# wustl-cig/FLAIR

Hardware: AMD Instinct MI355X
Metric: restored frames/sec at 256x256, 16-frame clip, 250-step DDIM (higher is better)
Workload: dtype bf16

## Files before the change

flair_amd/csrc/api.hip:

```cpp
#include <stdarg.h>
#include <stdio.h>

#include "common.h"

static thread_local char g_err[512] = "";

void flair_set_error(const char* fmt, ...) {
    va_list ap;
    va_start(ap, fmt);
    vsnprintf(g_err, sizeof(g_err), fmt, ap);
    va_end(ap);
}

extern "C" const char* flair_last_error(void) { return g_err; }
extern "C" int flair_abi_version(void) { return 11; }

#include <dlfcn.h>

typedef int (*flair_nccl_bcast_fn)(const void*, void*, size_t, int, int, void*, hipStream_t);

extern "C" int flair_bcast_weights(void* blob, size_t bytes, int root, void* rccl_comm, hipStream_t stream) {
    FLAIR_CHECK(blob && bytes > 0 && rccl_comm && root >= 0, "flair_bcast_weights: bad argument (blob, bytes, root, communicator)");
    static flair_nccl_bcast_fn fn = nullptr;
    if (!fn) {
        void* h = nullptr;
        for (const char* name : {"librccl.so", "librccl.so.1"}) {
            h = dlopen(name, RTLD_NOW | RTLD_NOLOAD);
            if (!h) h = dlopen(name, RTLD_NOW | RTLD_GLOBAL);
            if (h) break;
        }
        FLAIR_CHECK(h, "flair_bcast_weights: librccl.so not found (%s)", dlerror());
        fn = reinterpret_cast<flair_nccl_bcast_fn>(dlsym(h, "ncclBroadcast"));
        FLAIR_CHECK(fn, "flair_bcast_weights: ncclBroadcast not found in librccl");
    }
    const size_t chunk = (size_t)512 << 20;
    for (size_t off = 0; off < bytes; off += chunk) {
        const size_t n = bytes - off < chunk ? bytes - off : chunk;
        char* p = reinterpret_cast<char*>(blob) + off;
        const int rc = fn(p, p, n,  1, root, rccl_comm, stream);
        if (rc != 0) {
            flair_set_error("flair_bcast_weights: ncclBroadcast returned %d", rc);
            return FLAIR_ERR_HIP;
        }
    }
    return FLAIR_OK;
}

namespace {
typedef __attribute__((ext_vector_type(8))) __bf16 probe_bf16x8;
typedef __attribute__((ext_vector_type(16))) float probe_f32x16;

__global__ __launch_bounds__(256) void probe_matrix_kernel(float* sink, int iters) {
    probe_f32x16 acc[4];
    for (int i = 0; i < 4; ++i)
        for (int r = 0; r < 16; ++r) acc[i][r] = 0.f;
    probe_bf16x8 a, b;
    for (int e = 0; e < 8; ++e) {
        a[e] = (__bf16)(0.001f * (float)((threadIdx.x + e) & 255));
        b[e] = (__bf16)(0.002f * (float)((threadIdx.x + 2 * e) & 255));
    }
    for (int it = 0; it < iters; ++it) {
#pragma unroll
        for (int u = 0; u < 4; ++u)
#pragma unroll
            for (int i = 0; i < 4; ++i) acc[i] = __builtin_amdgcn_mfma_f32_32x32x16_bf16(a, b, acc[i], 0, 0, 0);
    }
    float s = 0.f;
    for (int i = 0; i < 4; ++i)
        for (int r = 0; r < 16; ++r) s += acc[i][r];
    if (s == 12345.678f) sink[0] = s;
}

__global__ __launch_bounds__(256) void probe_stream_kernel(const uint4* __restrict__ src, uint4* __restrict__ dst, size_t n, int mode) {
    unsigned sum = 0;
    for (size_t i = blockIdx.x * (size_t)blockDim.x + threadIdx.x; i < n; i += (size_t)gridDim.x * blockDim.x) {
        if (mode == 1) {
            dst[i] = make_uint4((unsigned)i, 1u, 2u, 3u);
        } else {
            const uint4 v = src[i];
            if (mode == 2) dst[i] = v;
            else sum ^= v.x ^ v.y ^ v.z ^ v.w;
        }
    }
    if (mode == 0 && sum == 0x12345679u) dst[0] = make_uint4(sum, 0u, 0u, 0u);
}
}

extern "C" int flair_probe_matrix_rate(int iters, int workgroups_per_cu, float* sink, double* flop_out, hipStream_t stream) {
    FLAIR_CHECK(iters > 0 && workgroups_per_cu >= 1 && workgroups_per_cu <= 8 && sink, "flair_probe_matrix_rate: bad argument");
    const int grid = flair_cu_count() * workgroups_per_cu;
    hipLaunchKernelGGL(probe_matrix_kernel, dim3(grid), dim3(256), 0, stream, sink, iters);
    FLAIR_LAUNCH_CHECK();
    if (flop_out) *flop_out = (double)grid * 4  * iters * 16  * (2.0 * 32 * 32 * 16);
    return FLAIR_OK;
}

extern "C" int flair_probe_stream_rate(const void* src, void* dst, size_t bytes, int mode, hipStream_t stream) {
    FLAIR_CHECK(dst && (mode == 1 || src) && bytes >= 16 && mode >= 0 && mode <= 2, "flair_probe_stream_rate: bad argument (mode 0 read, 1 write, 2 copy)");
    FLAIR_CHECK((reinterpret_cast<uintptr_t>(dst) & 15) == 0 && (reinterpret_cast<uintptr_t>(src) & 15) == 0, "flair_probe_stream_rate: 16-byte aligned buffers");
    hipLaunchKernelGGL(probe_stream_kernel, dim3(flair_cu_count() * 8), dim3(256), 0, stream, reinterpret_cast<const uint4*>(src),
                       reinterpret_cast<uint4*>(dst), bytes / 16, mode);
    FLAIR_LAUNCH_CHECK();
    return FLAIR_OK;
}
```

flair_amd/csrc/common.h:

```cpp
#pragma once
#include <hip/hip_runtime.h>
#include <stdint.h>

#include "../../include/flair_hip.h"

typedef __attribute__((ext_vector_type(8))) __bf16 bf16x8;
typedef __attribute__((ext_vector_type(16))) float f32x16;
typedef __attribute__((ext_vector_type(4))) float f32x4;

typedef uint16_t bf16_t;

#define FLAIR_WAVE 64

void flair_set_error(const char* fmt, ...);
#define FLAIR_CHECK(cond, ...)            \
    do {                                  \
        if (!(cond)) {                    \
            flair_set_error(__VA_ARGS__); \
            return FLAIR_ERR_ARG;         \
        }                                 \
    } while (0)
#define FLAIR_CHECK_VIEW(fn, name, ptr, ld, C, vec)                                                                   \
    FLAIR_CHECK((ld) >= (C) && (ld) % (vec) == 0 && reinterpret_cast<uintptr_t>(ptr) % 16 == 0,                        \
                fn ": " name " stride/alignment: " name "_ld = %d must be >= C = %d and a multiple of %d elements, " \
                name " = %p 16-byte aligned", (int)(ld), (int)(C), (int)(vec), (const void*)(ptr))
#define FLAIR_LAUNCH_CHECK()                                                  \
    do {                                                                      \
        hipError_t e_ = hipGetLastError();                                    \
        if (e_ != hipSuccess) {                                               \
            flair_set_error("HIP launch failed: %s", hipGetErrorString(e_));  \
            return FLAIR_ERR_HIP;                                             \
        }                                                                     \
    } while (0)

__device__ __forceinline__ float bf2f(bf16_t v) {
    return __uint_as_float(((uint32_t)v) << 16);
}
__device__ __forceinline__ bf16_t f2bf(float f) {
    __bf16 b = (__bf16)f;
    return __builtin_bit_cast(bf16_t, b);
}
__device__ __forceinline__ uint32_t pack2bf(float lo, float hi) {
    return (uint32_t)f2bf(lo) | ((uint32_t)f2bf(hi) << 16);
}

template <typename E> struct ET;
template <> struct ET<float> {
    static constexpr int VEC = 4;
    static constexpr int DT = FLAIR_F32;
    static __device__ __forceinline__ float ld(const float* p) { return *p; }
    static __device__ __forceinline__ void st(float* p, float v) { *p = v; }
};
template <> struct ET<bf16_t> {
    static constexpr int VEC = 8;
    static constexpr int DT = FLAIR_BF16;
    static __device__ __forceinline__ float ld(const bf16_t* p) { return bf2f(*p); }
    static __device__ __forceinline__ void st(bf16_t* p, float v) { *p = f2bf(v); }
};

template <typename E> struct Vec16;
template <> struct Vec16<float> {
    static __device__ __forceinline__ void load(const float* p, float* o) {
        float4 v = *reinterpret_cast<const float4*>(p);
        o[0] = v.x; o[1] = v.y; o[2] = v.z; o[3] = v.w;
    }
    static __device__ __forceinline__ void store(float* p, const float* o) {
        *reinterpret_cast<float4*>(p) = make_float4(o[0], o[1], o[2], o[3]);
    }
};
template <> struct Vec16<bf16_t> {
    static __device__ __forceinline__ void load(const bf16_t* p, float* o) {
        uint4 v = *reinterpret_cast<const uint4*>(p);
        o[0] = __uint_as_float(v.x << 16); o[1] = __uint_as_float(v.x & 0xffff0000u);
        o[2] = __uint_as_float(v.y << 16); o[3] = __uint_as_float(v.y & 0xffff0000u);
        o[4] = __uint_as_float(v.z << 16); o[5] = __uint_as_float(v.z & 0xffff0000u);
        o[6] = __uint_as_float(v.w << 16); o[7] = __uint_as_float(v.w & 0xffff0000u);
    }
    static __device__ __forceinline__ void store(bf16_t* p, const float* o) {
        uint4 v;
        v.x = pack2bf(o[0], o[1]); v.y = pack2bf(o[2], o[3]);
        v.z = pack2bf(o[4], o[5]); v.w = pack2bf(o[6], o[7]);
        *reinterpret_cast<uint4*>(p) = v;
    }
};

__device__ __forceinline__ float silu_f(float v) { return v / (1.0f + __expf(-v)); }

__device__ __forceinline__ float apply_act(float v, int act) {
    switch (act) {
        case FLAIR_ACT_RELU: return v > 0.f ? v : 0.f;
        case FLAIR_ACT_LRELU01: return v > 0.f ? v : 0.1f * v;
        case FLAIR_ACT_SILU: return silu_f(v);
        case FLAIR_ACT_LRELU02: return v > 0.f ? v : 0.2f * v;
        case FLAIR_ACT_GELU: return 0.5f * v * (1.f + erff(v * 0.70710678118654752f));
        default: return v;
    }
}

template <int N>
__device__ __forceinline__ void dcn_offset_act(float (&v)[N], int co, float mag, int period) {
    const bool residue = 3 * (co % period) < 2 * period;
#pragma unroll
    for (int e = 0; e < N; ++e) {
        const float r = __builtin_amdgcn_rcpf(1.f + __expf(residue ? 2.f * v[e] : -v[e]));
        v[e] = residue ? mag * (1.f - 2.f * r) : r;
    }
}

template <int N>
__device__ __forceinline__ void dcn_offset_act_fast(float (&v)[N], int co, float mag, int period, float scale) {
    const bool residue = 3 * (co % period) < 2 * period;
    const float kk = residue ? 2.885390081777927f : -1.4426950408889634f;
    const float A = residue ? -2.f * mag * scale : scale, B = residue ? mag * scale : 0.f;
#pragma unroll
    for (int e = 0; e < N; ++e) v[e] = fmaf(__builtin_amdgcn_rcpf(1.f + __builtin_amdgcn_exp2f(kk * v[e])), A, B);
}

typedef __attribute__((ext_vector_type(4))) unsigned int u32x4_t;
#define FLAIR_OOB 0x80000000u
__device__ __forceinline__ __amdgpu_buffer_rsrc_t make_rsrc(const void* p, unsigned bytes) {
    return __builtin_amdgcn_make_buffer_rsrc(const_cast<void*>(p), 0, (int)bytes, 0x00020000);
}
__device__ __forceinline__ uint4 buf_load16(__amdgpu_buffer_rsrc_t r, unsigned byteOff) {
    const u32x4_t v = __builtin_amdgcn_raw_buffer_load_b128(r, (int)byteOff, 0, 0);
    return make_uint4(v.x, v.y, v.z, v.w);
}

__device__ __forceinline__ int xcd_remap(int bid, int nwg) {
    const int q = nwg >> 3, r = nwg & 7, xcd = bid & 7;
    const int base = xcd < r ? xcd * (q + 1) : r * (q + 1) + (xcd - r) * q;
    return base + (bid >> 3);
}

template <int NBYTES>
__device__ __forceinline__ void prefetch_kernargs() {
#ifdef FLAIR_NO_KARG_PREFETCH
    return;
#endif
    const auto ka = __builtin_amdgcn_kernarg_segment_ptr();
    constexpr int LINES = (NBYTES + 63) / 64 + 1;
    unsigned t0, t1, t2, t3, t4, t5, t6, t7;
    if constexpr (LINES <= 2)
        asm volatile("s_load_dword %0, %2, 0x0\n\ts_load_dword %1, %2, 0x40\n\ts_waitcnt lgkmcnt(0)" : "=&s"(t0), "=&s"(t1) : "s"(ka) : "memory");
    else if constexpr (LINES <= 4)
        asm volatile("s_load_dword %0, %4, 0x0\n\ts_load_dword %1, %4, 0x40\n\ts_load_dword %2, %4, 0x80\n\ts_load_dword %3, %4, 0xc0\n\t"
                     "s_waitcnt lgkmcnt(0)" : "=&s"(t0), "=&s"(t1), "=&s"(t2), "=&s"(t3) : "s"(ka) : "memory");
    else if constexpr (LINES <= 6)
        asm volatile("s_load_dword %0, %6, 0x0\n\ts_load_dword %1, %6, 0x40\n\ts_load_dword %2, %6, 0x80\n\ts_load_dword %3, %6, 0xc0\n\t"
                     "s_load_dword %4, %6, 0x100\n\ts_load_dword %5, %6, 0x140\n\ts_waitcnt lgkmcnt(0)"
                     : "=&s"(t0), "=&s"(t1), "=&s"(t2), "=&s"(t3), "=&s"(t4), "=&s"(t5) : "s"(ka) : "memory");
    else
        asm volatile("s_load_dword %0, %8, 0x0\n\ts_load_dword %1, %8, 0x40\n\ts_load_dword %2, %8, 0x80\n\ts_load_dword %3, %8, 0xc0\n\t"
                     "s_load_dword %4, %8, 0x100\n\ts_load_dword %5, %8, 0x140\n\ts_load_dword %6, %8, 0x180\n\ts_load_dword %7, %8, 0x1c0\n\t"
                     "s_waitcnt lgkmcnt(0)"
                     : "=&s"(t0), "=&s"(t1), "=&s"(t2), "=&s"(t3), "=&s"(t4), "=&s"(t5), "=&s"(t6), "=&s"(t7) : "s"(ka) : "memory");
}

__device__ __forceinline__ void dma16(u32x4_t desc, unsigned voff, unsigned ldsAddr) {
    unsigned keep;
    asm volatile("s_mov_b32 %0, m0\n\ts_mov_b32 m0, %2\n\ts_nop 0\n\tbuffer_load_dwordx4 %1, %3, 0 offen lds\n\ts_mov_b32 m0, %0"
                 : "=&s"(keep)
                 : "v"(voff), "s"(ldsAddr), "s"(desc)
                 : "memory");
}

__device__ __forceinline__ u32x4_t make_desc(const void* base, unsigned bytes) {
    const unsigned long long b = reinterpret_cast<unsigned long long>(base);
    u32x4_t d;
    d.x = __builtin_amdgcn_readfirstlane((unsigned)b);
    d.y = __builtin_amdgcn_readfirstlane((unsigned)(b >> 32) & 0xffffu);
    d.z = __builtin_amdgcn_readfirstlane(bytes);
    d.w = 0x00020000u;
    return d;
}

struct LdsAttrOnce {
    unsigned long long done = 0;
};
static inline hipError_t flair_max_lds_once(LdsAttrOnce& st, const void* fn, int bytes = 160 * 1024) {
    int dev = 0;
    if (hipGetDevice(&dev) != hipSuccess) dev = -1;
    if (dev >= 0 && dev < 64 && ((st.done >> dev) & 1ull)) return hipSuccess;
    const hipError_t e = hipFuncSetAttribute(fn, hipFuncAttributeMaxDynamicSharedMemorySize, bytes);
    if (e == hipSuccess && dev >= 0 && dev < 64) st.done |= 1ull << dev;
    return e;
}
static inline int flair_cu_count() {
    static int cus[64] = {};
    int dev = 0;
    if (hipGetDevice(&dev) != hipSuccess || dev < 0 || dev >= 64) return 256;
    if (!cus[dev]) {
        hipDeviceProp_t prop;
        cus[dev] = hipGetDeviceProperties(&prop, dev) == hipSuccess && prop.multiProcessorCount > 0 ? prop.multiProcessorCount : 256;
    }
    return cus[dev];
}

static inline int cdiv(long a, long b) { return (int)((a + b - 1) / b); }
```

flair_amd/csrc/conv.hip:

```cpp
#include <type_traits>

#include "common.h"

namespace {

struct ConvArgs {
    const void* x[4];
    int segC[4];
    int segLd[4];
    int nseg;
    const void* w;
    const float* bias;
    const void* res0;
    const void* res1;
    int res0Ld, res1Ld;
    void* y;
    int yLd;
    int T, H, W;
    int KT, KH, KW;
    int Cout, CinTot;
    int act;
    float outScale;
    long P;
    int nPixTiles, nCoTiles;
    int tFast;
    unsigned segBytes[4];
    unsigned wBytes;
    float* part;
    int splitK;
    const float* fbias;
    int fbiasLd;
    int stride;
    int tapShift;
    int reflect;
    float actParam;
    int actPeriod;
    int Hin, Win;
    int esz;
};

template <typename E> struct Mma;

template <> struct Mma<bf16_t> {
    static constexpr int BKE = 32;
    static __device__ __forceinline__ int chunk(int i, int half) { return 2 * i + half; }
    static __device__ __forceinline__ void run(const uint4 (&a)[2], const uint4 (&b)[2], f32x16& acc) {
        acc = __builtin_amdgcn_mfma_f32_32x32x16_bf16(__builtin_bit_cast(bf16x8, a[0]),
                                                      __builtin_bit_cast(bf16x8, b[0]), acc, 0, 0, 0);
        acc = __builtin_amdgcn_mfma_f32_32x32x16_bf16(__builtin_bit_cast(bf16x8, a[1]),
                                                      __builtin_bit_cast(bf16x8, b[1]), acc, 0, 0, 0);
    }
    static __device__ __forceinline__ void run1(const uint4& a, const uint4& b, f32x16& acc) {
        acc = __builtin_amdgcn_mfma_f32_32x32x16_bf16(__builtin_bit_cast(bf16x8, a), __builtin_bit_cast(bf16x8, b),
                                                      acc, 0, 0, 0);
    }
    static constexpr int MFMA_PER_HALF = 1;
};

template <> struct Mma<float> {
    static constexpr int BKE = 16;
    static __device__ __forceinline__ int chunk(int i, int half) { return 2 * half + i; }
    static __device__ __forceinline__ void run(const uint4 (&a)[2], const uint4 (&b)[2], f32x16& acc) {
        const float* af = reinterpret_cast<const float*>(a);
        const float* bf = reinterpret_cast<const float*>(b);
#pragma unroll
        for (int s = 0; s < 8; ++s)
            acc = __builtin_amdgcn_mfma_f32_32x32x2f32(af[s], bf[s], acc, 0, 0, 0);
    }
    static __device__ __forceinline__ void run1(const uint4& a, const uint4& b, f32x16& acc) {
        const float* af = reinterpret_cast<const float*>(&a);
        const float* bf = reinterpret_cast<const float*>(&b);
#pragma unroll
        for (int s = 0; s < 4; ++s)
            acc = __builtin_amdgcn_mfma_f32_32x32x2f32(af[s], bf[s], acc, 0, 0, 0);
    }
    static constexpr int MFMA_PER_HALF = 4;
};

__device__ __forceinline__ int lds_off(int row, int chunk) {
    return row * 64 + ((chunk ^ ((row >> 2) & 3)) << 4);
}

__device__ __forceinline__ int staged_row(int id) {
    const int g = id >> 3;
    return (g >> 2) * 8 + (g & 3) + 4 * ((id >> 2) & 1);
}

template <typename E>
__device__ __forceinline__ void store_quad(const ConvArgs& a, long p, int co, float v0, float v1, float v2, float v3) {
    if (co >= a.Cout) return;
    float v[4] = {v0, v1, v2, v3};
    if (a.bias) {
        const float4 b = *reinterpret_cast<const float4*>(a.bias + co);
        v[0] += b.x; v[1] += b.y; v[2] += b.z; v[3] += b.w;
    }
    if (a.fbias) {
        const float* fb = a.fbias + (p / ((long)a.H * a.W)) * a.fbiasLd + co;
        v[0] += fb[0]; v[1] += fb[1]; v[2] += fb[2]; v[3] += fb[3];
    }
    if (a.act == FLAIR_ACT_DCN_OFFSETS) {
        dcn_offset_act<4>(v, co, a.actParam, a.actPeriod);
    } else {
#pragma unroll
        for (int e = 0; e < 4; ++e) v[e] = apply_act(v[e], a.act);
    }
    const E* r0 = reinterpret_cast<const E*>(a.res0);
    const E* r1 = reinterpret_cast<const E*>(a.res1);
    if (r0) {
#pragma unroll
        for (int e = 0; e < 4; ++e) v[e] += ET<E>::ld(r0 + p * a.res0Ld + co + e);
    }
    if (r1) {
#pragma unroll
        for (int e = 0; e < 4; ++e) v[e] += ET<E>::ld(r1 + p * a.res1Ld + co + e);
    }
#pragma unroll
    for (int e = 0; e < 4; ++e) v[e] *= a.outScale;
    E* dst = reinterpret_cast<E*>(a.y) + p * a.yLd + co;
    if constexpr (sizeof(E) == 4) {
        *reinterpret_cast<float4*>(dst) = make_float4(v[0], v[1], v[2], v[3]);
    } else {
        uint2 pk;
        pk.x = pack2bf(v[0], v[1]);
        pk.y = pack2bf(v[2], v[3]);
        *reinterpret_cast<uint2*>(dst) = pk;
    }
}

template <typename E, int ACT, int FC, int FP>
__device__ __forceinline__ void igemm_epilogue(const ConvArgs& a, const f32x16 (&acc)[FC][FP], long pbase, int cobase, int lr, int lh) {
    constexpr unsigned ESZ = sizeof(E);
    constexpr int VEC = ET<E>::VEC, NV = 8 / VEC;
    const float slope = a.act == FLAIR_ACT_NONE ? 1.f : a.act == FLAIR_ACT_RELU ? 0.f : a.act == FLAIR_ACT_LRELU01 ? 0.1f : 0.2f;
    const unsigned yLdB = (unsigned)a.yLd * ESZ, r0LdB = (unsigned)a.res0Ld * ESZ, r1LdB = (unsigned)a.res1Ld * ESZ;
    constexpr unsigned SPAN = FP * 32;
    const __amdgpu_buffer_rsrc_t yd = make_rsrc(reinterpret_cast<char*>(a.y) + ((size_t)pbase * a.yLd + cobase) * ESZ, SPAN * yLdB);
    const __amdgpu_buffer_rsrc_t r0d = make_rsrc(reinterpret_cast<const char*>(a.res0) + (a.res0 ? ((size_t)pbase * a.res0Ld + cobase) * ESZ : 0),
                                                 a.res0 ? SPAN * r0LdB : 0u);
    const __amdgpu_buffer_rsrc_t r1d = make_rsrc(reinterpret_cast<const char*>(a.res1) + (a.res1 ? ((size_t)pbase * a.res1Ld + cobase) * ESZ : 0),
                                                 a.res1 ? SPAN * r1LdB : 0u);
    const int coLeft = a.Cout - cobase;
    const __amdgpu_buffer_rsrc_t bd = make_rsrc(a.bias ? a.bias + cobase : nullptr, a.bias && coLeft > 0 ? (unsigned)coLeft * 4u : 0u);
    const long hw = (long)a.H * a.W;
#pragma unroll
    for (int j = 0; j < FP; ++j) {
        const long p = pbase + j * 32 + lr;
        const bool pvalid = p < a.P;
        const unsigned pl = (unsigned)(j * 32 + lr);
        const float* fbrow = a.fbias ? a.fbias + (pvalid ? p / hw : 0) * a.fbiasLd + cobase : nullptr;
#pragma unroll
        for (int i = 0; i < FC; ++i) {
            uint4 bq[2][2], r0v[2][NV], r1v[2][NV], fq[2][2];
#pragma unroll
            for (int jj = 0; jj < 2; ++jj) {
                const int cw = i * 32 + 16 * jj + 8 * lh;
                const bool ok = pvalid && cw < coLeft;
                bq[jj][0] = buf_load16(bd, 4u * (unsigned)cw);
                bq[jj][1] = buf_load16(bd, 4u * (unsigned)cw + 16u);
#pragma unroll
                for (int q = 0; q < NV; ++q) {
                    r0v[jj][q] = buf_load16(r0d, ok ? pl * r0LdB + (unsigned)(cw + q * VEC) * ESZ : FLAIR_OOB);
                    r1v[jj][q] = buf_load16(r1d, ok ? pl * r1LdB + (unsigned)(cw + q * VEC) * ESZ : FLAIR_OOB);
                }
                fq[jj][0] = fq[jj][1] = make_uint4(0u, 0u, 0u, 0u);
            }
            if (a.fbias) {
#pragma unroll
                for (int jj = 0; jj < 2; ++jj) {
                    const int cw = i * 32 + 16 * jj + 8 * lh;
                    const float* fp = fbrow + (cw < coLeft ? cw : 0);
                    fq[jj][0] = *reinterpret_cast<const uint4*>(fp);
                    fq[jj][1] = *reinterpret_cast<const uint4*>(fp + 4);
                }
            }
#pragma unroll
            for (int jj = 0; jj < 2; ++jj) {
                const f32x16& c = acc[i][j];
                float v[8];
#pragma unroll
                for (int e = 0; e < 4; ++e) {
                    const auto sw2 = __builtin_amdgcn_permlane32_swap(__float_as_uint(c[8 * jj + e]), __float_as_uint(c[8 * jj + 4 + e]), false, false);
                    v[e] = __uint_as_float(sw2[0]);
                    v[4 + e] = __uint_as_float(sw2[1]);
                }
                const int cw = i * 32 + 16 * jj + 8 * lh;
                const bool ok = pvalid && cw < coLeft;
                {
                    const uint4 b0 = bq[jj][0], b1 = bq[jj][1], f0 = fq[jj][0], f1 = fq[jj][1];
                    v[0] += __uint_as_float(b0.x) + __uint_as_float(f0.x); v[1] += __uint_as_float(b0.y) + __uint_as_float(f0.y);
                    v[2] += __uint_as_float(b0.z) + __uint_as_float(f0.z); v[3] += __uint_as_float(b0.w) + __uint_as_float(f0.w);
                    v[4] += __uint_as_float(b1.x) + __uint_as_float(f1.x); v[5] += __uint_as_float(b1.y) + __uint_as_float(f1.y);
                    v[6] += __uint_as_float(b1.z) + __uint_as_float(f1.z); v[7] += __uint_as_float(b1.w) + __uint_as_float(f1.w);
                }
// ... 157 lines not shown
            fa0[set][0] = *reinterpret_cast<const uint4*>(wb0 + tap9 * PITCH + 16 * Mma<E>::chunk(0, lh));
            fa0[set][1] = *reinterpret_cast<const uint4*>(wb0 + tap9 * PITCH + 16 * Mma<E>::chunk(1, lh));
            fa1[set][0] = *reinterpret_cast<const uint4*>(wb1 + tap9 * PITCH + 16 * Mma<E>::chunk(0, lh));
            fa1[set][1] = *reinterpret_cast<const uint4*>(wb1 + tap9 * PITCH + 16 * Mma<E>::chunk(1, lh));
#pragma unroll
            for (int j = 0; j < RPW; ++j) {
                const char* hp = hb + ((j + kh) * HW_ + kw) * PITCH;
                fb[set][j][0] = *reinterpret_cast<const uint4*>(hp + 16 * Mma<E>::chunk(0, lh));
                fb[set][j][1] = *reinterpret_cast<const uint4*>(hp + 16 * Mma<E>::chunk(1, lh));
            }
        };
        load_tap(0, 0);
        __builtin_amdgcn_sched_group_barrier(0x100, 4 + 2 * RPW, 0);
#pragma unroll
        for (int tap9 = 0; tap9 < 9; ++tap9) {
            const int set = tap9 & 1;
            if (tap9 < 8) load_tap(set ^ 1, tap9 + 1);
#pragma unroll
            for (int j = 0; j < RPW; ++j) {
                Mma<E>::run(fa0[set], fb[set][j], acc[j][0]);
                Mma<E>::run(fa1[set], fb[set][j], acc[j][1]);
            }
            if (tap9 < 8) __builtin_amdgcn_sched_group_barrier(0x100, 4 + 2 * RPW, 0);
            __builtin_amdgcn_sched_group_barrier(0x8, (sizeof(E) == 2 ? 4 : 16) * RPW, 0);
        }
    };

    int issued = 0;
#pragma unroll
    for (int s_ = 0; s_ < PF; ++s_)
        if (issued < nch) {
            issue(hreg[s_], wreg[s_]);
            advance();
            ++issued;
        }
    write_lds(hreg[0], wreg[0]);
    __syncthreads();
    for (int k = 0; k < nch; k += PF) {
#pragma unroll
        for (int par = 0; par < PF; ++par) {
            const int kk = k + par;
            if (kk < nch) {
                if (issued < nch) {
                    issue(hreg[par], wreg[par]);
                    advance();
                    ++issued;
                }
                compute();
                if (kk + 1 < nch) {
                    __syncthreads();
                    write_lds(hreg[(par + 1) % PF], wreg[(par + 1) % PF]);
                    __syncthreads();
                }
            }
        }
    }

    if ((a.Cout & 7) == 0) {
        constexpr int VEC = ET<E>::VEC;
        constexpr int CHUNKS = 64 / VEC;
        __syncthreads();
#pragma unroll
        for (int j = 0; j < RPW; ++j) {
            char* tile = smem + (wave * RPW + j) * 32 * (64 * 4 + 16);
#pragma unroll
            for (int i = 0; i < 2; ++i)
#pragma unroll
                for (int g = 0; g < 4; ++g)
                    *reinterpret_cast<float4*>(tile + lr * (64 * 4 + 16) + (i * 32 + 8 * g + 4 * lh) * 4) =
                        make_float4(acc[j][i][4 * g], acc[j][i][4 * g + 1], acc[j][i][4 * g + 2],
                                    acc[j][i][4 * g + 3]);
        }
        __syncthreads();
        constexpr int FPITCH = 64 * 4 + 16;
#pragma unroll
        for (int j = 0; j < RPW; ++j) {
            const int h = h0 + wave * RPW + j;
            if (h >= a.H) continue;
            const char* tile = smem + (wave * RPW + j) * 32 * FPITCH;
            const long prow = ((long)t * a.H + h) * a.W + w0;
#pragma unroll
            for (int it = 0; it < 32 * CHUNKS / 64; ++it) {
                const int id = it * 64 + lane;
                const int px = id / CHUNKS, ch = id % CHUNKS;
                const int co = co0 + ch * VEC;
                if (co >= a.Cout) continue;
                const long p = prow + px;
                float v[VEC];
                const float* src = reinterpret_cast<const float*>(tile + px * FPITCH) + ch * VEC;
#pragma unroll
                for (int e = 0; e < VEC; e += 4) {
                    const float4 q = *reinterpret_cast<const float4*>(src + e);
                    v[e] = q.x; v[e + 1] = q.y; v[e + 2] = q.z; v[e + 3] = q.w;
                }
                if (a.bias) {
#pragma unroll
                    for (int e = 0; e < VEC; ++e) v[e] += a.bias[co + e];
                }
                if (a.fbias) {
                    const float* fb = a.fbias + (long)t * a.fbiasLd + co;
#pragma unroll
                    for (int e = 0; e < VEC; ++e) v[e] += fb[e];
                }
                if (a.act == FLAIR_ACT_DCN_OFFSETS) {
                    dcn_offset_act<VEC>(v, co, a.actParam, a.actPeriod);
                } else {
#pragma unroll
                    for (int e = 0; e < VEC; ++e) v[e] = apply_act(v[e], a.act);
                }
                if (a.res0) {
                    float r[VEC];
                    Vec16<E>::load(reinterpret_cast<const E*>(a.res0) + p * a.res0Ld + co, r);
#pragma unroll
                    for (int e = 0; e < VEC; ++e) v[e] += r[e];
                }
                if (a.res1) {
                    float r[VEC];
                    Vec16<E>::load(reinterpret_cast<const E*>(a.res1) + p * a.res1Ld + co, r);
#pragma unroll
                    for (int e = 0; e < VEC; ++e) v[e] += r[e];
                }
#pragma unroll
                for (int e = 0; e < VEC; ++e) v[e] *= a.outScale;
                Vec16<E>::store(reinterpret_cast<E*>(a.y) + p * a.yLd + co, v);
            }
        }
        return;
    }
#pragma unroll
    for (int j = 0; j < RPW; ++j) {
        const int h = h0 + wave * RPW + j, w = w0 + lr;
        if (h >= a.H) continue;
        const long p = ((long)t * a.H + h) * a.W + w;
#pragma unroll
        for (int i = 0; i < 2; ++i)
#pragma unroll
            for (int g = 0; g < 4; ++g)
                store_quad<E>(a, p, co0 + i * 32 + 8 * g + 4 * lh, acc[j][i][4 * g], acc[j][i][4 * g + 1],
                              acc[j][i][4 * g + 2], acc[j][i][4 * g + 3]);
    }
}

template <typename E, int TH, int RPW, int PF>
int launch_halo(const ConvArgs& a0, hipStream_t s) {
    ConvArgs a = a0;
    a.nCoTiles = cdiv(a.Cout, 64);
    const int grid = a.T * cdiv(a.H, TH) * (a.W / 32) * a.nCoTiles;
    const size_t lds = (size_t)(TH + 2) * 34 * 80 + 64 * 9 * 80;
    hipLaunchKernelGGL((conv3x3_halo_kernel<E, TH, RPW, PF>), dim3(grid), dim3(64 * TH / RPW), lds, s, a);
    FLAIR_LAUNCH_CHECK();
    return FLAIR_OK;
}

template <typename E, int TH, int RPW, int CF>
__global__ __launch_bounds__(256 * TH / RPW / CF, (256 * TH / RPW / CF) / 256) void conv3x3_halo_ks_kernel(ConvArgs a) {
    static_assert(RPW == 1 && CF == 2, "one image row and both 32-cout fragments per wave");
    prefetch_kernargs<sizeof(ConvArgs)>();
    constexpr int NRG = TH / RPW;
    constexpr int NCG = 2 / CF;
    constexpr int NW = 2 * NRG * NCG, NT = 64 * NW;
    constexpr int BKE = Mma<E>::BKE;
    constexpr int VEC = ET<E>::VEC;
    constexpr unsigned ESZ = sizeof(E);
    constexpr int HW_ = 34, PITCH = 80;
    constexpr int HALO_ROWS = (TH + 2) * HW_;
    constexpr int HALO_PIECES = (HALO_ROWS + 7) / 8 * 8 * 4;
    constexpr int W_PIECES = 64 * 9 * 4;
    constexpr int HI = (HALO_PIECES + NT - 1) / NT;
    constexpr int WI = (W_PIECES + NT - 1) / NT;
    constexpr int HALO_BYTES = (TH + 2) * HW_ * PITCH;
    constexpr int STAGE_BYTES = HALO_BYTES + 64 * 9 * PITCH;
    extern __shared__ __attribute__((aligned(16))) char smem[];

    const int tid = threadIdx.x, lane = tid & 63, wave = tid >> 6;
    const int lr = lane & 31, lh = lane >> 5;
    const int rp = wave % NRG, kh2 = (wave / NRG) & 1, cg = wave / (2 * NRG);
    const int bid = xcd_remap(blockIdx.x, gridDim.x);
    const int coTile = bid % a.nCoTiles;
    int rest = bid / a.nCoTiles;
    const int tilesW = a.W / 32, tilesH = (a.H + TH - 1) / TH;
    const int tw = rest % tilesW;
    rest /= tilesW;
    const int th = rest % tilesH;
    const int t = rest / tilesH;
    const int h0 = th * TH, w0 = tw * 32, co0 = coTile * 64;
    const int taps = a.KT * 9;
    const int pt = a.KT / 2;

    float biasv[VEC];
    {
        const int bco = co0 + (lane % (64 / VEC)) * VEC;
#pragma unroll
        for (int e = 0; e < VEC; ++e) biasv[e] = (a.bias && bco < a.Cout) ? a.bias[bco + e] : 0.f;
    }
    uint4 hreg[HI], wreg[WI];
    int dt = -pt, seg = 0, cb = 0, segOff = 0;
    auto dt_valid = [&](int d) { return (unsigned)(t + d) < (unsigned)a.T; };
    while (dt <= pt && !dt_valid(dt)) ++dt;

    int hpix[HI];
    unsigned hq[HI], woff[WI];
#pragma unroll
    for (int i = 0; i < HI; ++i) {
        const int id = i * NT + tid;
        const int pix = staged_row(id);
        const int r = pix / HW_, c = pix % HW_;
        const int hh = h0 + r - 1, ww = w0 + c - 1;
        const bool ok = pix < HALO_ROWS && (unsigned)hh < (unsigned)a.H && (unsigned)ww < (unsigned)a.W;
        hpix[i] = ok ? hh * a.W + ww : -1;
        hq[i] = (id & 3) * VEC * ESZ;
    }
    const __amdgpu_buffer_rsrc_t wrs = make_rsrc(a.w, a.wBytes);
#pragma unroll
    for (int i = 0; i < WI; ++i) {
        const int id = i * NT + tid;
        const int row = staged_row(id);
        const int co = row / 9, tap9 = row % 9;
        const bool ok = id < W_PIECES && co0 + co < a.Cout;
        woff[i] = ok ? (unsigned)(((co0 + co) * taps + tap9) * a.CinTot + (id & 3) * VEC) * ESZ : FLAIR_OOB;
    }
    auto issue = [&]() {
        const unsigned ld = (unsigned)a.segLd[seg] * ESZ;
        const char* frame = reinterpret_cast<const char*>(a.x[seg]) + (size_t)(t + dt) * a.H * a.W * ld;
        const __amdgpu_buffer_rsrc_t xr = make_rsrc(frame, a.segBytes[seg]);
        const unsigned cofs = (unsigned)(cb * BKE) * ESZ;
#pragma unroll
        for (int i = 0; i < HI; ++i)
            hreg[i] = buf_load16(xr, hpix[i] >= 0 ? (unsigned)hpix[i] * ld + cofs + hq[i] : FLAIR_OOB);
        const unsigned kofs = (unsigned)((dt + pt) * 9 * a.CinTot + segOff + cb * BKE) * ESZ;
#pragma unroll
        for (int i = 0; i < WI; ++i) wreg[i] = buf_load16(wrs, woff[i] == FLAIR_OOB ? FLAIR_OOB : woff[i] + kofs);
        ++cb;
        if (cb * BKE >= a.segC[seg]) {
            cb = 0;
            segOff += a.segC[seg];
            if (++seg >= a.nseg) {
                seg = 0;
                segOff = 0;
                ++dt;
                while (dt <= pt && !dt_valid(dt)) ++dt;
            }
        }
    };
    auto write_lds = [&](int stage) {
        char* sh = smem + stage * STAGE_BYTES;
        char* sw = sh + HALO_BYTES;
#pragma unroll
        for (int i = 0; i < HI; ++i) {
            const int id = i * NT + tid;
            const int row = staged_row(id);
            if (row < HALO_ROWS) *reinterpret_cast<uint4*>(sh + row * PITCH + (id & 3) * 16) = hreg[i];
        }
#pragma unroll
        for (int i = 0; i < WI; ++i) {
            const int id = i * NT + tid;
            if (id < W_PIECES) *reinterpret_cast<uint4*>(sw + staged_row(id) * PITCH + (id & 3) * 16) = wreg[i];
        }
    };
    int nValidDt = 0;
    for (int d = -pt; d <= pt; ++d) nValidDt += dt_valid(d) ? 1 : 0;
    const int nch = nValidDt * (a.CinTot / BKE);

    f32x16 acc[RPW][CF];
#pragma unroll
    for (int j = 0; j < RPW; ++j)
#pragma unroll
        for (int i = 0; i < CF; ++i)
#pragma unroll
            for (int r = 0; r < 16; ++r) acc[j][i][r] = 0.f;

    const int ck = 16 * Mma<E>::chunk(kh2, lh);
    auto compute = [&](int stage) {
        const char* sh = smem + stage * STAGE_BYTES;
        const char* hb = sh + ((RPW * rp * HW_) + lr) * PITCH + ck;
        const char* wb0 = sh + HALO_BYTES + ((cg * CF * 32 + lr) * 9) * PITCH + ck;
        uint4 fa[2][CF], fb[2][RPW];
        auto load_tap = [&](int set, int tap9) {
            const int kh = tap9 / 3, kw = tap9 % 3;
#pragma unroll
            for (int i = 0; i < CF; ++i)
                fa[set][i] = *reinterpret_cast<const uint4*>(wb0 + (i * 32 * 9 + tap9) * PITCH);
#pragma unroll
            for (int j = 0; j < RPW; ++j)
                fb[set][j] = *reinterpret_cast<const uint4*>(hb + ((kh + j) * HW_ + kw) * PITCH);
        };
        load_tap(0, 0);
        __builtin_amdgcn_sched_group_barrier(0x100, CF + RPW, 0);
#pragma unroll
        for (int tap9 = 0; tap9 < 9; ++tap9) {
            const int set = tap9 & 1;
            if (tap9 < 8) load_tap(set ^ 1, tap9 + 1);
#pragma unroll
            for (int j = 0; j < RPW; ++j)
#pragma unroll
                for (int i = 0; i < CF; ++i) Mma<E>::run1(fa[set][i], fb[set][j], acc[j][i]);
            if (tap9 < 8) __builtin_amdgcn_sched_group_barrier(0x100, CF + RPW, 0);
            __builtin_amdgcn_sched_group_barrier(0x8, CF * RPW * Mma<E>::MFMA_PER_HALF, 0);
        }
    };

    issue();
    write_lds(0);
    if (nch > 1) issue();
    __syncthreads();
    for (int k = 0; k < nch; ++k) {
        compute(k & 1);
        if (k + 1 < nch) {
            write_lds((k + 1) & 1);
            if (k + 2 < nch) issue();
            __syncthreads();
        }
    }

    constexpr int FPITCH = 64 * 4 + 16;
    constexpr int CHUNKS = 64 / VEC;
    constexpr int PARTS = NW / TH;
    constexpr int NIT = 32 * CHUNKS / 64 / PARTS;
    const int orow = wave % TH, part = wave / TH;
    const int h = h0 + orow;
    const long prow = ((long)t * a.H + h) * a.W + w0;
    const int ech = lane % CHUNKS;
    const int eco = co0 + ech * VEC;
    const bool eok = h < a.H && eco < a.Cout;
    uint4 r0v[NIT], r1v[NIT];
#pragma unroll
    for (int k = 0; k < NIT; ++k) {
        const int px = ((k * PARTS + part) * 64 + lane) / CHUNKS;
        const long p = prow + px;
        r0v[k] = r1v[k] = make_uint4(0u, 0u, 0u, 0u);
        if (eok && a.res0) r0v[k] = *reinterpret_cast<const uint4*>(reinterpret_cast<const E*>(a.res0) + p * a.res0Ld + eco);
        if (eok && a.res1) r1v[k] = *reinterpret_cast<const uint4*>(reinterpret_cast<const E*>(a.res1) + p * a.res1Ld + eco);
    }
    __syncthreads();
#pragma unroll
    for (int pass = 0; pass < 2; ++pass) {
        if (kh2 == pass) {
#pragma unroll
            for (int j = 0; j < RPW; ++j) {
                char* tile = smem + (RPW * rp + j) * 32 * FPITCH + lr * FPITCH;
#pragma unroll
                for (int i = 0; i < CF; ++i)
#pragma unroll
                    for (int g = 0; g < 4; ++g) {
                        float4* dst = reinterpret_cast<float4*>(tile + ((cg * CF + i) * 32 + 8 * g + 4 * lh) * 4);
                        float4 v = make_float4(acc[j][i][4 * g], acc[j][i][4 * g + 1], acc[j][i][4 * g + 2],
                                               acc[j][i][4 * g + 3]);
                        if (pass == 1) {
                            const float4 o = *dst;
                            v.x += o.x; v.y += o.y; v.z += o.z; v.w += o.w;
                        }
                        *dst = v;
                    }
            }
        }
        __syncthreads();
    }
    if (!eok) return;
    const float slope = a.act == FLAIR_ACT_NONE ? 1.f : a.act == FLAIR_ACT_RELU ? 0.f : a.act == FLAIR_ACT_LRELU01 ? 0.1f : 0.2f;
    const bool leaky = a.act == FLAIR_ACT_NONE || a.act == FLAIR_ACT_RELU || a.act == FLAIR_ACT_LRELU01 || a.act == FLAIR_ACT_LRELU02;
    const char* tile = smem + orow * 32 * FPITCH;
#pragma unroll
    for (int k = 0; k < NIT; ++k) {
        const int px = ((k * PARTS + part) * 64 + lane) / CHUNKS;
        const long p = prow + px;
        float v[VEC];
        const float* src = reinterpret_cast<const float*>(tile + px * FPITCH) + ech * VEC;
#pragma unroll
        for (int e = 0; e < VEC; e += 4) {
            const float4 q = *reinterpret_cast<const float4*>(src + e);
            v[e] = q.x; v[e + 1] = q.y; v[e + 2] = q.z; v[e + 3] = q.w;
        }
#pragma unroll
        for (int e = 0; e < VEC; ++e) v[e] += biasv[e];
        if (a.fbias) {
            const float* fb = a.fbias + (long)t * a.fbiasLd + eco;
#pragma unroll
            for (int e = 0; e < VEC; ++e) v[e] += fb[e];
        }
        if (leaky) {
#pragma unroll
            for (int e = 0; e < VEC; ++e) v[e] = fmaxf(v[e], v[e] * slope);
        } else if (a.act == FLAIR_ACT_DCN_OFFSETS) {
            dcn_offset_act<VEC>(v, eco, a.actParam, a.actPeriod);
        } else if (a.act == FLAIR_ACT_SILU) {
#pragma unroll
            for (int e = 0; e < VEC; ++e) v[e] = silu_f(v[e]);
        } else {
#pragma unroll
            for (int e = 0; e < VEC; ++e) v[e] = apply_act(v[e], a.act);
        }
        if (a.res0) {
            float r[VEC];
            Vec16<E>::load(reinterpret_cast<const E*>(&r0v[k]), r);
#pragma unroll
            for (int e = 0; e < VEC; ++e) v[e] += r[e];
        }
        if (a.res1) {
            float r[VEC];
            Vec16<E>::load(reinterpret_cast<const E*>(&r1v[k]), r);
#pragma unroll
            for (int e = 0; e < VEC; ++e) v[e] += r[e];
        }
#pragma unroll
        for (int e = 0; e < VEC; ++e) v[e] *= a.outScale;
        Vec16<E>::store(reinterpret_cast<E*>(a.y) + p * a.yLd + eco, v);
    }
}

template <typename E, int TH, int RPW, int CF>
int launch_halo_ks(const ConvArgs& a0, hipStream_t s) {
    ConvArgs a = a0;
    a.nCoTiles = cdiv(a.Cout, 64);
    const int grid = a.T * cdiv(a.H, TH) * (a.W / 32) * a.nCoTiles;
    const size_t lds = 2 * ((size_t)(TH + 2) * 34 * 80 + 64 * 9 * 80);
    static LdsAttrOnce attr;
    {
        const hipError_t e = flair_max_lds_once(attr, reinterpret_cast<const void*>(&conv3x3_halo_ks_kernel<E, TH, RPW, CF>));
        FLAIR_CHECK(e == hipSuccess, "flair_conv_nhwc: hipFuncSetAttribute: %s", hipGetErrorString(e));
    }
    hipLaunchKernelGGL((conv3x3_halo_ks_kernel<E, TH, RPW, CF>), dim3(grid), dim3(256 * TH / RPW / CF), lds, s, a);
    FLAIR_LAUNCH_CHECK();
    return FLAIR_OK;
}

struct DmaTile {
    int t, h0, w0, co0;
};

template <int NW, int RPW, int NSTAGE>
__device__ __forceinline__ void conv3x3_dma_body(const ConvArgs& a, int nTiles, int tilesPerXcd) {
    using E = bf16_t;
    static_assert((RPW == 1 || RPW == 2) && NSTAGE == 2, "the clip-level and one-tile forms (two stages)");
    constexpr int KSTEPS = 2;
    constexpr int TH = NW * RPW, HWP = 34;
    constexpr int HALO_ROWS = (TH + 2) * HWP;
    constexpr int HALO_INSTR = (HALO_ROWS + 15) / 16;
    constexpr int W_INSTR = 64 * 9 / 16;
    constexpr int HALO_BYTES = HALO_INSTR * 1024;
    constexpr int STAGE_BYTES = HALO_BYTES + W_INSTR * 1024;
    constexpr int NSLOT = (HALO_INSTR + W_INSTR + NW - 1) / NW;
    constexpr int BIAS_OFF = NSTAGE * STAGE_BYTES + NW * 1024;
    extern __shared__ __attribute__((aligned(16))) char smem[];

    const int tid = threadIdx.x, lane = tid & 63;
    const int wave = __builtin_amdgcn_readfirstlane(tid >> 6);
    const int lr = lane & 31, lh = lane >> 5;
    const int taps = a.KT * 9, pt = a.KT / 2;
    const int chunksPerTap = a.CinTot / 32;
    const int H = a.H, W = a.W, T = a.T;

    const int xcd = blockIdx.x & 7, slot = blockIdx.x >> 3, slotsPerXcd = gridDim.x >> 3;
    const int tilesW = W / 32, tilesH = H / TH, nCoTiles = a.nCoTiles;
    auto tile_at = [&](int i, DmaTile& tl) -> bool {
        const int inXcd = slot + i * slotsPerXcd;
        const int id = xcd * tilesPerXcd + inXcd;
        if (inXcd >= tilesPerXcd || id >= nTiles) return false;
        int rest = id;
        tl.co0 = (rest % nCoTiles) * 64;
        rest /= nCoTiles;
        if (a.tFast) {
            tl.t = rest % T;
            rest /= T;
            tl.w0 = (rest % tilesW) * 32;
            tl.h0 = (rest / tilesW) * TH;
            return true;
        }
        tl.w0 = (rest % tilesW) * 32;
        rest /= tilesW;
        tl.h0 = (rest % tilesH) * TH;
        tl.t = rest / tilesH;
        return true;
    };

    const int lrow = lane >> 2, lchunk = lane & 3;
    unsigned slotv[NSLOT], hchunk[NSLOT];
#pragma unroll
    for (int i = 0; i < NSLOT; ++i) {
        const int id = wave * NSLOT + i;
        const int c = (id * 16 + lrow) % HWP;
        hchunk[i] = (unsigned)((lchunk ^ ((c >> 2) & 3)) << 4);
    }
    auto setup_tile = [&](const DmaTile& tl) {
#pragma unroll
        for (int i = 0; i < NSLOT; ++i) {
            const int id = wave * NSLOT + i;
            const int R = id * 16 + lrow;
            const int hr = R / HWP, c = R - hr * HWP;
            const int hh = tl.h0 - 1 + hr, ww = tl.w0 - 1 + c;
            const bool okh = R < HALO_ROWS && (unsigned)hh < (unsigned)H && (unsigned)ww < (unsigned)W;
            const unsigned hv = okh ? (unsigned)(hh * W + ww) : 0xffffffffu;
            const int row = R - HALO_INSTR * 16;
            const int tap9 = row >> 6, co = row & 63;
            const bool okw = row >= 0 && row < 576 && tl.co0 + co < a.Cout;
            const unsigned wv = okw ? (unsigned)(((tl.co0 + co) * taps + tap9) * a.CinTot) * 2u + ((lchunk ^ ((co >> 2) & 3)) << 4) : FLAIR_OOB;
            slotv[i] = id >= HALO_INSTR ? wv : hv;
        }
    };

    const u32x4_t wdesc = make_desc(a.w, a.wBytes);
    struct Walk {
        int dt, seg, cb, segOff, j;
    };
    auto dt_at = [&](int t, int j) { return a.tFast ? (j + a.KT * T - t) % a.KT - pt : j - pt; };
    auto walk_first = [&](int t, Walk& wk) {
        wk.j = 0; wk.seg = 0; wk.cb = 0; wk.segOff = 0;
        while (wk.j < a.KT && (unsigned)(t + dt_at(t, wk.j)) >= (unsigned)T) ++wk.j;
        wk.dt = dt_at(t, wk.j);
    };
    auto walk_next = [&](int t, Walk& wk) {
        ++wk.cb;
        if (wk.cb * 32 >= a.segC[wk.seg]) {
            wk.cb = 0;
            wk.segOff += a.segC[wk.seg];
            if (++wk.seg >= a.nseg) {
                wk.seg = 0;
                wk.segOff = 0;
                ++wk.j;
                while (wk.j < a.KT && (unsigned)(t + dt_at(t, wk.j)) >= (unsigned)T) ++wk.j;
                wk.dt = dt_at(t, wk.j);
            }
        }
    };
    auto chunks_of = [&](int t) {
        int n = 0;
        for (int d = -pt; d <= pt; ++d) n += (unsigned)(t + d) < (unsigned)T ? 1 : 0;
        return n * chunksPerTap;
    };
    auto issue = [&](const DmaTile& tl, const Walk& wk, int stage) {
        const unsigned ld = (unsigned)a.segLd[wk.seg] * 2u;
        const char* frame = reinterpret_cast<const char*>(a.x[wk.seg]) + (size_t)(tl.t + wk.dt) * H * W * ld;
        const u32x4_t xdesc = make_desc(frame, a.segBytes[wk.seg]);
        const unsigned cofs = (unsigned)(wk.cb * 64);
        const unsigned kofs = (unsigned)((wk.dt + pt) * 9 * a.CinTot + wk.segOff + wk.cb * 32) * 2u;
        const unsigned sbase = (unsigned)(stage * STAGE_BYTES + wave * NSLOT * 1024);
#pragma unroll
        for (int i = 0; i < NSLOT; ++i) {
            const bool isw = wave * NSLOT + i >= HALO_INSTR;
            const unsigned sv = slotv[i];
            const unsigned offh = sv == 0xffffffffu ? FLAIR_OOB : sv * ld + cofs + hchunk[i];
            const unsigned offw = sv == FLAIR_OOB ? FLAIR_OOB : sv + kofs;
            u32x4_t d;
            d.x = isw ? wdesc.x : xdesc.x;
            d.y = isw ? wdesc.y : xdesc.y;
            d.z = isw ? wdesc.z : xdesc.z;
            d.w = 0x00020000u;
            const bool idle = wave * NSLOT + i >= HALO_INSTR + W_INSTR;
            dma16(d, isw ? offw : offh, idle ? (unsigned)(NSTAGE * STAGE_BYTES + ((wave * NSLOT + i - HALO_INSTR - W_INSTR) % NW) * 1024) : sbase + i * 1024);
        }
    };

    unsigned aoff[KSTEPS], boff[3][KSTEPS];
#pragma unroll
    for (int s_ = 0; s_ < KSTEPS; ++s_) {
        aoff[s_] = (unsigned)(HALO_BYTES + lr * 64 + (((2 * s_ + lh) ^ ((lr >> 2) & 3)) << 4));
#pragma unroll
        for (int kw = 0; kw < 3; ++kw)
            boff[kw][s_] = (unsigned)((RPW * wave * HWP + kw + lr) * 64 + (((2 * s_ + lh) ^ (((kw + lr) >> 2) & 3)) << 4));
    }

// ... 164 lines not shown
                        v[e] = __uint_as_float(sw2[0]) + bv[e];
                        v[4 + e] = __uint_as_float(sw2[1]) + bv[4 + e];
                    }
                    if constexpr (ACT == 0) {
#pragma unroll
                        for (int e = 0; e < 8; ++e) v[e] = fmaxf(v[e], v[e] * slope);
                    } else if constexpr (ACT == 1) {
                        dcn_offset_act<8>(v, tl.co0 + cofs + cl, a.actParam, a.actPeriod);
                    } else {
#pragma unroll
                        for (int e = 0; e < 8; ++e) v[e] = silu_f(v[e]);
                    }
                    const long ro = (long)j * W;
                    if (r0b && lane_ok) {
                        float r[8];
                        Vec16<E>::load(r0b + ro * a.res0Ld + cofs, r);
#pragma unroll
                        for (int e = 0; e < 8; ++e) v[e] += r[e];
                    }
                    if (r1b && lane_ok) {
                        float r[8];
                        Vec16<E>::load(r1b + ro * a.res1Ld + cofs, r);
#pragma unroll
                        for (int e = 0; e < 8; ++e) v[e] += r[e];
                    }
#pragma unroll
                    for (int e = 0; e < 8; ++e) v[e] *= scale;
                    if (!lane_ok) continue;
                    Vec16<E>::store(yb + ro * a.yLd + cofs, v);
                }
            }
    };
    auto epilogue = [&](const DmaTile& tl, int biasSlot) {
        const bool res = a.res0 || a.res1;
        auto go = [&](auto actTag) {
            if constexpr (RPW == 1) {
                epilogue_plain_as(tl, biasSlot, actTag);
            } else {
                if (res) epilogue_as(tl, biasSlot, actTag, std::true_type{});
                else epilogue_as(tl, biasSlot, actTag, std::false_type{});
            }
        };
        if (a.act == FLAIR_ACT_DCN_OFFSETS) go(std::integral_constant<int, 1>{});
        else if (a.act == FLAIR_ACT_SILU) go(std::integral_constant<int, 2>{});
        else if (RPW >= 2 && a.act == FLAIR_ACT_NONE && a.outScale == 1.f) go(std::integral_constant<int, 3>{});
        else go(std::integral_constant<int, 0>{});
    };

    DmaTile cur, nxt;
    int iCur = 0, iNxt = 0;
    if (!tile_at(0, cur)) return;
    nxt = cur;
    Walk wk;
    walk_first(nxt.t, wk);
    setup_tile(nxt);
    float4 biasReg = make_float4(0.f, 0.f, 0.f, 0.f);
    bool biasPending = false;
    auto bias_request = [&](const DmaTile& tl) {
        if (tid < 16) {
            const int bco = tl.co0 + 4 * tid;
            biasReg = (a.bias && bco < a.Cout) ? *reinterpret_cast<const float4*>(a.bias + bco) : make_float4(0.f, 0.f, 0.f, 0.f);
            if (a.fbias && bco < a.Cout) {
                const float* fb = a.fbias + (long)tl.t * a.fbiasLd + bco;
                biasReg.x += fb[0]; biasReg.y += fb[1]; biasReg.z += fb[2]; biasReg.w += fb[3];
            }
        }
        biasPending = true;
    };
    auto bias_commit = [&](int slot_) {
        if (tid < 16) *reinterpret_cast<float4*>(smem + BIAS_OFF + (slot_ & 1) * 256 + 16 * tid) = biasReg;
        biasPending = false;
    };
    bias_request(nxt);
    bias_commit(0);
    const bool res0any = a.res0 || a.res1;
    int remIssue = chunks_of(nxt.t);
    int remCompute = remIssue;
    bool more = true;
    int stage = 0;
    issue(nxt, wk, 0);
    walk_next(nxt.t, wk);
    --remIssue;
    asm volatile("s_waitcnt vmcnt(0)" ::: "memory");
    __syncthreads();
    zero_acc();
    while (true) {
        if (more && remIssue == 0) {
            ++iNxt;
            more = tile_at(iNxt, nxt);
            if (more) {
                walk_first(nxt.t, wk);
                setup_tile(nxt);
                remIssue = chunks_of(nxt.t);
                bias_request(nxt);
            }
        }
        if (more) {
            issue(nxt, wk, stage ^ 1);
            walk_next(nxt.t, wk);
            --remIssue;
        }
        compute(stage);
        if (biasPending) bias_commit(iNxt);
        bool storesInFlight = false;
        if (--remCompute == 0) {
            epilogue(cur, iCur);
            storesInFlight = RPW >= 2 ? !a.res1 : cur.co0 + 64 <= a.Cout && !res0any;
            ++iCur;
            if (!tile_at(iCur, cur)) break;
            remCompute = chunks_of(cur.t);
            zero_acc();
        }
        if (storesInFlight) {
            asm volatile("s_waitcnt vmcnt(%0)" ::"n"(4 * RPW) : "memory");
        } else {
            asm volatile("s_waitcnt vmcnt(0)" ::: "memory");
        }
        __syncthreads();
        stage ^= 1;
    }
}

template <int NW, int RPW, int NSTAGE>
__global__ __launch_bounds__(64 * NW, (NW + 3) / 4) void conv3x3_dma_kernel(ConvArgs a, int nTiles, int tilesPerXcd) {
    prefetch_kernargs<sizeof(ConvArgs) + 8>();
    conv3x3_dma_body<NW, RPW, NSTAGE>(a, nTiles, tilesPerXcd);
}

template <int NW, int RPW, int NSTAGE>
int launch_dma(const ConvArgs& a0, hipStream_t s) {
    constexpr int TH = NW * RPW;
    ConvArgs a = a0;
    a.nCoTiles = cdiv(a.Cout, 64);
    a.tFast = a.KT == 3 && a.T > 1;
    const int nTiles = a.T * (a.H / TH) * (a.W / 32) * a.nCoTiles;
    const int nCu = flair_cu_count();
    int grid = nTiles < nCu ? (nTiles + 7) / 8 * 8 : nCu / 8 * 8;
    if (grid < 8) grid = 8;
    const int tilesPerXcd = (nTiles + 7) / 8;
    constexpr int HALO_INSTR = ((TH + 2) * 34 + 15) / 16;
    const size_t lds = NSTAGE * (size_t)(HALO_INSTR + 36) * 1024 + NW * 1024 + 512;
    static LdsAttrOnce attr;
    {
        const hipError_t e = flair_max_lds_once(attr, reinterpret_cast<const void*>(&conv3x3_dma_kernel<NW, RPW, NSTAGE>));
        FLAIR_CHECK(e == hipSuccess, "flair_conv_nhwc: hipFuncSetAttribute: %s", hipGetErrorString(e));
    }
    hipLaunchKernelGGL((conv3x3_dma_kernel<NW, RPW, NSTAGE>), dim3(grid), dim3(64 * NW), lds, s, a, nTiles, tilesPerXcd);

    FLAIR_LAUNCH_CHECK();
    return FLAIR_OK;
}


template <bool HALO3>
__global__ __launch_bounds__(512, 2) void conv_frame_kernel(ConvArgs a) {
    static_assert(HALO3, "halo ring of three, weight ring of two");
    prefetch_kernargs<sizeof(ConvArgs)>();
    using E = bf16_t;
    constexpr int NW = 8, HWP = 34;
    constexpr int HINSTR = 22, HIMG = HINSTR * 1024, WINSTR = 36, SLOT = WINSTR * 1024;
    constexpr int HR = 3, WR = 2;
    constexpr int RING = HR * HIMG, BIAS = RING + WR * SLOT;
    constexpr int NH = (HINSTR + NW - 1) / NW, NWS = (WINSTR + NW - 1) / NW;
    extern __shared__ __attribute__((aligned(16))) char smem[];
    const int tid = threadIdx.x, lane = tid & 63;
    const int wave = __builtin_amdgcn_readfirstlane(tid >> 6);
    const int lr = lane & 31, lh = lane >> 5;
    const int lrow = lane >> 2, lchunk = lane & 3;
    const int tilesW = a.W / 32, perFrame = tilesW * (a.H / 8);
    const int bid = xcd_remap(blockIdx.x, gridDim.x);
    const int t = bid / perFrame, tile = bid - t * perFrame;
    const int h0 = (tile / tilesW) * 8, w0 = (tile % tilesW) * 32;
    const int nS = a.CinTot / 32;

    const u32x4_t wdesc = make_desc(a.w, a.wBytes);
    const u32x4_t bdesc = make_desc(a.bias, a.bias ? (unsigned)a.Cout * 4u : 0u);
    dma16(bdesc, (unsigned)(lane * 16), (unsigned)BIAS);
    unsigned hpix[NH], hpiece[NH];
#pragma unroll
    for (int i = 0; i < NH; ++i) {
        const int k = (wave * NH + i) % HINSTR;
        const int R = k * 16 + lrow;
        const int hr = R / HWP, c = R - hr * HWP;
        const int hh = h0 - 1 + hr, ww = w0 - 1 + c;
        const bool ok = R < 10 * HWP && (unsigned)hh < (unsigned)a.H && (unsigned)ww < (unsigned)a.W;
        hpix[i] = ok ? (unsigned)(hh * a.W + ww) : 0xffffffffu;
        hpiece[i] = (unsigned)((lchunk ^ ((c >> 2) & 3)) << 4);
    }
    unsigned wlane[NWS];
#pragma unroll
    for (int i = 0; i < NWS; ++i) {
        const int id = (wave * NWS + i) % WINSTR;
        const int row = id * 16 + lrow, tap9 = row >> 6, co = row & 63;
        wlane[i] = co < a.Cout ? (unsigned)((co * 9 + tap9) * a.CinTot) * 2u + (unsigned)((lchunk ^ ((co >> 2) & 3)) << 4) : FLAIR_OOB;
    }
    int hseg = 0, hcb = 0;
    auto issue_halo = [&](int slot) {
        const unsigned ld = (unsigned)a.segLd[hseg] * 2u;
        const u32x4_t xdesc = make_desc(reinterpret_cast<const char*>(a.x[hseg]) + (size_t)t * a.H * a.W * ld, a.segBytes[hseg]);
        const unsigned cofs = (unsigned)(hcb * 64);
#pragma unroll
        for (int i = 0; i < NH; ++i) {
            const int k = (wave * NH + i) % HINSTR;
            dma16(xdesc, hpix[i] == 0xffffffffu ? FLAIR_OOB : hpix[i] * ld + cofs + hpiece[i], (unsigned)(slot * HIMG + k * 1024));
        }
        if (++hcb * 32 >= a.segC[hseg]) {
            hcb = 0;
            ++hseg;
        }
    };
    auto issue_w = [&](int s_) {
#pragma unroll
        for (int i = 0; i < NWS; ++i) {
            const int id = (wave * NWS + i) % WINSTR;
            dma16(wdesc, wlane[i] == FLAIR_OOB ? FLAIR_OOB : wlane[i] + (unsigned)(s_ * 64), (unsigned)(RING + (s_ % WR) * SLOT + id * 1024));
        }
    };
    issue_halo(0);
    issue_w(0);
    if (nS > 1) {
        issue_halo(1);
        issue_w(1);
    }
    if (nS > 2) issue_halo(2);

    unsigned aoff[2], boff[3][2];
#pragma unroll
    for (int ks = 0; ks < 2; ++ks) {
        aoff[ks] = (unsigned)(lr * 64 + (((2 * ks + lh) ^ ((lr >> 2) & 3)) << 4));
#pragma unroll
        for (int kw = 0; kw < 3; ++kw)
            boff[kw][ks] = (unsigned)((wave * HWP + kw + lr) * 64 + (((2 * ks + lh) ^ (((kw + lr) >> 2) & 3)) << 4));
    }
    f32x16 acc[2];
    auto compute = [&](int wslot, int hslot) {
        const char* wb = smem + RING + wslot * SLOT;
        const char* xb = smem + hslot * HIMG;
        uint4 fb[2][3][2], fa[2][2][2];
        auto load_b = [&](int set, int kw) {
#pragma unroll
            for (int h = 0; h < 3; ++h)
#pragma unroll
                for (int ks = 0; ks < 2; ++ks) fb[set][h][ks] = *reinterpret_cast<const uint4*>(xb + h * (HWP * 64) + boff[kw][ks]);
        };
        auto load_a = [&](int set, int kh, int kw) {
#pragma unroll
            for (int cf = 0; cf < 2; ++cf)
#pragma unroll
                for (int ks = 0; ks < 2; ++ks) fa[set][cf][ks] = *reinterpret_cast<const uint4*>(wb + (kh * 3 + kw) * 4096 + cf * 2048 + aoff[ks]);
        };
        load_b(0, 0);
        load_a(0, 0, 0);
#pragma unroll
        for (int step = 0; step < 9; ++step) {
            const int kq = step / 3, kh = step % 3;
            const int nkq = (step + 1) / 3, nkh = (step + 1) % 3;
            if (step < 8) {
                if (nkh == 0) load_b(nkq & 1, nkq);
                load_a((step + 1) & 1, nkh, nkq);
            }
#pragma unroll
            for (int cf = 0; cf < 2; ++cf)
#pragma unroll
                for (int ks = 0; ks < 2; ++ks)
                    acc[cf] = __builtin_amdgcn_mfma_f32_32x32x16_bf16(__builtin_bit_cast(bf16x8, fa[step & 1][cf][ks]), __builtin_bit_cast(bf16x8, fb[kq & 1][kh][ks]), acc[cf], 0, 0, 0);
        }
    };

    const long prow = ((long)t * a.H + h0 + wave) * a.W + w0;
    const unsigned yLdB = (unsigned)a.yLd * 2u, r0LdB = (unsigned)a.res0Ld * 2u, r1LdB = (unsigned)a.res1Ld * 2u;
    const __amdgpu_buffer_rsrc_t yd = make_rsrc(reinterpret_cast<char*>(a.y) + prow * a.yLd * 2, (unsigned)a.W * yLdB);
    const __amdgpu_buffer_rsrc_t r0d = make_rsrc(a.res0 ? reinterpret_cast<const char*>(a.res0) + prow * a.res0Ld * 2 : nullptr, a.res0 ? (unsigned)a.W * r0LdB : 0u);
    const __amdgpu_buffer_rsrc_t r1d = make_rsrc(a.res1 ? reinterpret_cast<const char*>(a.res1) + prow * a.res1Ld * 2 : nullptr, a.res1 ? (unsigned)a.W * r1LdB : 0u);
    uint4 r0v[4], r1v[4];
#pragma unroll
    for (int g = 0; g < 4; ++g) r0v[g] = r1v[g] = make_uint4(0u, 0u, 0u, 0u);

    for (int s_ = 0; s_ < nS; ++s_) {
        if (s_ + 1 >= nS) asm volatile("s_waitcnt vmcnt(0)" ::: "memory");
        else if (s_ == 0 && nS > 2) asm volatile("s_waitcnt vmcnt(%0)" ::"n"(2 * NH + NWS) : "memory");
        else if (s_ == 0) asm volatile("s_waitcnt vmcnt(%0)" ::"n"(NH + NWS) : "memory");
        else asm volatile("s_waitcnt vmcnt(%0)" ::"n"(NH) : "memory");
        __builtin_amdgcn_s_barrier();
        if (s_ == 0) {
            const float* sb = reinterpret_cast<const float*>(smem + BIAS);
#pragma unroll
            for (int cf = 0; cf < 2; ++cf)
#pragma unroll
                for (int g = 0; g < 4; ++g) {
                    const float4 bq = *reinterpret_cast<const float4*>(sb + cf * 32 + 8 * g + 4 * lh);
                    acc[cf][4 * g] = bq.x; acc[cf][4 * g + 1] = bq.y; acc[cf][4 * g + 2] = bq.z; acc[cf][4 * g + 3] = bq.w;
                }
        }
        if (s_ >= 1 && s_ + 1 < nS) issue_w(s_ + 1);
        if (s_ >= 1 && s_ + 2 < nS) issue_halo((s_ + 2) % 3);
        if (s_ + 1 == nS) {
            if (a.res0) {
#pragma unroll
                for (int g = 0; g < 4; ++g) r0v[g] = buf_load16(r0d, 16 * g + 8 * lh < a.Cout ? (unsigned)lr * r0LdB + (unsigned)(32 * g + 16 * lh) : FLAIR_OOB);
            }
            if (a.res1) {
#pragma unroll
                for (int g = 0; g < 4; ++g) r1v[g] = buf_load16(r1d, 16 * g + 8 * lh < a.Cout ? (unsigned)lr * r1LdB + (unsigned)(32 * g + 16 * lh) : FLAIR_OOB);
            }
        }
        compute(s_ % WR, s_ % HR);
    }

    const float slope = a.act == FLAIR_ACT_NONE ? 1.f : a.act == FLAIR_ACT_RELU ? 0.f : a.act == FLAIR_ACT_LRELU01 ? 0.1f : 0.2f;
    const float scale = a.outScale;
#pragma unroll
    for (int cf = 0; cf < 2; ++cf)
#pragma unroll
        for (int jj = 0; jj < 2; ++jj) {
            const int g = 2 * cf + jj;
            float v[8];
#pragma unroll
            for (int e = 0; e < 4; ++e) {
                const auto sw2 = __builtin_amdgcn_permlane32_swap(__float_as_uint(acc[cf][8 * jj + e]), __float_as_uint(acc[cf][8 * jj + 4 + e]), false, false);
                v[e] = __uint_as_float(sw2[0]);
                v[4 + e] = __uint_as_float(sw2[1]);
            }
#pragma unroll
            for (int e = 0; e < 8; ++e) v[e] = fmaxf(v[e], v[e] * slope);
            float r[8];
            Vec16<E>::load(reinterpret_cast<const E*>(&r0v[g]), r);
#pragma unroll
            for (int e = 0; e < 8; ++e) v[e] += r[e];
            Vec16<E>::load(reinterpret_cast<const E*>(&r1v[g]), r);
#pragma unroll
            for (int e = 0; e < 8; ++e) v[e] = (v[e] + r[e]) * scale;
            alignas(16) E out[8];
            Vec16<E>::store(out, v);
            const uint4 ov = *reinterpret_cast<const uint4*>(out);
            const unsigned yo = 16 * g + 8 * lh < a.Cout ? (unsigned)lr * yLdB + (unsigned)(32 * g + 16 * lh) : FLAIR_OOB;
            __builtin_amdgcn_raw_buffer_store_b128(u32x4_t{ov.x, ov.y, ov.z, ov.w}, yd, (int)yo, 0, 0);
        }
}

static bool frame_kernel_ok(const ConvArgs& a) {
    if (a.esz != 2 || a.KT != 1 || a.KH != 3 || a.KW != 3 || a.stride != 1 || a.fbias || a.Cout > 64 || a.Cout % 8 || a.W % 32 || a.H % 8) return false;
    if (!(a.act == FLAIR_ACT_NONE || a.act == FLAIR_ACT_RELU || a.act == FLAIR_ACT_LRELU01 || a.act == FLAIR_ACT_LRELU02)) return false;
    if (a.tapShift || a.reflect || a.CinTot % 32 || a.CinTot < 32) return false;
    for (int i = 0; i < a.nseg; ++i)
        if (a.segC[i] % 32) return false;
    return true;
}

static int launch_frame(const ConvArgs& a, hipStream_t s) {
    constexpr size_t lds = (3 * 22 + 2 * 36) * 1024 + 1024;
    static LdsAttrOnce attr;
    const hipError_t e = flair_max_lds_once(attr, reinterpret_cast<const void*>(&conv_frame_kernel<true>));
    FLAIR_CHECK(e == hipSuccess, "flair_conv_nhwc: hipFuncSetAttribute: %s", hipGetErrorString(e));
    hipLaunchKernelGGL(conv_frame_kernel<true>, dim3(a.T * (a.H / 8) * (a.W / 32)), dim3(512), lds, s, a);
    FLAIR_LAUNCH_CHECK();
    return FLAIR_OK;
}

template <typename E, int TC, int TP, int WC, int WP, int PD, int KWID>
__global__ __launch_bounds__(256) void conv_igemm_kernel(ConvArgs a) {
    prefetch_kernargs<sizeof(ConvArgs)>();
    constexpr int BKE = Mma<E>::BKE * KWID;
    constexpr int ROWB = 64 * KWID;
    constexpr int CPR = 4 * KWID;
    constexpr int RPP = 256 / CPR;
    constexpr int VEC = ET<E>::VEC;
    constexpr int FC = TC / WC / 32;
    constexpr int FP = TP / WP / 32;
    constexpr int XR = TP / RPP;
    constexpr int WR = TC / RPP;
    static_assert(WC * WP == 4 && FC >= 1 && FP >= 1 && XR >= 1 && WR >= 1, "tile");

    extern __shared__ __attribute__((aligned(16))) char smem[];
    constexpr int BUF = (TC + TP) * ROWB;
    auto loff = [](int row, int chunk) { return KWID == 1 ? lds_off(row, chunk) : row * 128 + ((chunk ^ ((row >> 1) & 7)) << 4); };

    const int tid = threadIdx.x;
    const int lane = tid & 63, wave = __builtin_amdgcn_readfirstlane(tid >> 6);
    const int wc = wave / WP, wp = wave % WP;

    const int bid = xcd_remap(blockIdx.x, gridDim.x);
    const int coTile = bid % a.nCoTiles;
    const int pixTile = bid / a.nCoTiles;
    const long p0 = (long)pixTile * TP;
    const int co0 = coTile * TC;

    const int chunk = tid % CPR;
    const int srow = tid / CPR;
    int xt[XR], xh[XR], xw[XR];
    bool xvalid[XR];
#pragma unroll
    for (int i = 0; i < XR; ++i) {
        long p = p0 + srow + RPP * i;
        xvalid[i] = p < a.P;
        if (!xvalid[i]) p = 0;
        int w_ = (int)(p % a.W);
        long q = p / a.W;
        xw[i] = w_;
        xh[i] = (int)(q % a.H);
        xt[i] = (int)(q / a.H);
    }
    const int taps = a.KT * a.KH * a.KW;
    const int pt = a.KT / 2, ph = a.KH / 2, pw = a.KW / 2;
    const int tFirst = (int)(p0 / ((long)a.H * a.W));
    const int tileFrames = (int)((TP + (long)a.H * a.W - 1) / ((long)a.H * a.W)) + 1;

    uint4 xreg[PD][XR], wreg[PD][WR];

    const int nkAll = taps * (a.CinTot / BKE);
    const int ks0 = (int)((long)blockIdx.y * nkAll / a.splitK);
    const int ks1 = (int)((long)(blockIdx.y + 1) * nkAll / a.splitK);
    int tap = ks0 / (a.CinTot / BKE), seg = 0, cb = ks0 % (a.CinTot / BKE), segOff = 0;
    while (cb * BKE >= a.segC[seg]) {
        cb -= a.segC[seg] / BKE;
        segOff += a.segC[seg];
        ++seg;
    }
    int dw = tap % a.KW - pw, dh = (tap / a.KW) % a.KH - ph, dt = tap / (a.KW * a.KH) - pt;

    const __amdgpu_buffer_rsrc_t wrs = make_rsrc(a.w, a.wBytes);
    constexpr unsigned ESZ = sizeof(E);
    auto issue_loads = [&](int set) {
        const int ld = a.segLd[seg];
        int fb = tFirst + dt;
        fb = fb < 0 ? 0 : (fb >= a.T ? a.T - 1 : fb);
        int nfr = a.T - fb;
        if (nfr > tileFrames) nfr = tileFrames;
        const size_t frameBytes = (size_t)a.Hin * a.Win * ld * ESZ;
        const __amdgpu_buffer_rsrc_t xr =
            make_rsrc(reinterpret_cast<const char*>(a.x[seg]) + fb * frameBytes, (unsigned)(nfr * frameBytes));
        const int coff = cb * BKE + chunk * VEC;
#pragma unroll
        for (int i = 0; i < XR; ++i) {
            const int t2 = xt[i] + dt;
            int h2 = xh[i] * a.stride + dh + a.tapShift, w2 = xw[i] * a.stride + dw + a.tapShift;
            if (a.reflect) {
                h2 = h2 < 0 ? -h2 : (h2 >= a.Hin ? 2 * a.Hin - 2 - h2 : h2);
                w2 = w2 < 0 ? -w2 : (w2 >= a.Win ? 2 * a.Win - 2 - w2 : w2);
            }
            const bool ok = xvalid[i] && (unsigned)t2 < (unsigned)a.T && (unsigned)h2 < (unsigned)a.Hin &&
                            (unsigned)w2 < (unsigned)a.Win;
            const unsigned off = ok ? (unsigned)((((t2 - fb) * a.Hin + h2) * a.Win + w2) * ld + coff) * ESZ : FLAIR_OOB;
            xreg[set][i] = buf_load16(xr, off);
        }
        const unsigned kofs = (unsigned)(tap * a.CinTot + segOff + coff) * ESZ;
#pragma unroll
        for (int j = 0; j < WR; ++j) {
            const int n = co0 + srow + RPP * j;
            wreg[set][j] = buf_load16(wrs, n < a.Cout ? (unsigned)(n * taps * a.CinTot) * ESZ + kofs : FLAIR_OOB);
        }
    };
    auto advance = [&]() {
        ++cb;
        if (cb * BKE >= a.segC[seg]) {
            cb = 0;
            segOff += a.segC[seg];
            ++seg;
            if (seg >= a.nseg) {
                seg = 0;
                segOff = 0;
                ++tap;
                ++dw;
                if (dw > pw) {
                    dw = -pw;
                    ++dh;
                    if (dh > ph) {
                        dh = -ph;
                        ++dt;
                    }
                }
            }
        }
    };
    auto write_lds = [&](int buf, int set) {
        char* base = smem + buf * BUF;
#pragma unroll
        for (int j = 0; j < WR; ++j)
            *reinterpret_cast<uint4*>(base + loff(srow + RPP * j, chunk)) = wreg[set][j];
#pragma unroll
        for (int i = 0; i < XR; ++i)
            *reinterpret_cast<uint4*>(base + TC * ROWB + loff(srow + RPP * i, chunk)) = xreg[set][i];
    };

    f32x16 acc[FC][FP];
#pragma unroll
    for (int i = 0; i < FC; ++i)
#pragma unroll
        for (int j = 0; j < FP; ++j)
#pragma unroll
            for (int r = 0; r < 16; ++r) acc[i][j][r] = 0.f;

    const int nk = ks1 - ks0;
    const int lr = lane & 31, lh = lane >> 5;

#pragma unroll
    for (int u = 0; u < PD; ++u)
        if (u < nk) {
            issue_loads(u);
            advance();
        }
    write_lds(0, 0);
    __syncthreads();

    for (int ks = 0; ks < nk; ks += PD) {
#pragma unroll
        for (int u = 0; u < PD; ++u) {
            const int k = ks + u;
// ... 60 lines not shown
        else run(std::integral_constant<int, 0>{});
        return;
    }
#pragma unroll
    for (int j = 0; j < FP; ++j) {
        const long p = p0 + wp * (TP / WP) + j * 32 + lr;
        if (p >= a.P) continue;
#pragma unroll
        for (int i = 0; i < FC; ++i)
#pragma unroll
            for (int g = 0; g < 4; ++g)
                store_quad<E>(a, p, co0 + wc * (TC / WC) + i * 32 + 8 * g + 4 * lh, acc[i][j][4 * g],
                              acc[i][j][4 * g + 1], acc[i][j][4 * g + 2], acc[i][j][4 * g + 3]);
    }
}

template <typename E>
__global__ void conv_splitk_reduce_kernel(ConvArgs a) {
    const unsigned cq = (unsigned)(a.Cout / 4);
    const unsigned quads = (unsigned)a.P * cq;
    const size_t slice = (size_t)a.P * a.Cout;
    for (unsigned i = blockIdx.x * blockDim.x + threadIdx.x; i < quads; i += gridDim.x * blockDim.x) {
        const unsigned p = i / cq;
        const int co = (int)(i - p * cq) * 4;
        const float* src = a.part + (size_t)p * a.Cout + co;
        float4 s = make_float4(0.f, 0.f, 0.f, 0.f);
        int k = 0;
        for (; k + 4 <= a.splitK; k += 4) {
            float4 v[4];
#pragma unroll
            for (int u = 0; u < 4; ++u) v[u] = *reinterpret_cast<const float4*>(src + (size_t)(k + u) * slice);
#pragma unroll
            for (int u = 0; u < 4; ++u) {
                s.x += v[u].x; s.y += v[u].y; s.z += v[u].z; s.w += v[u].w;
            }
        }
        for (; k < a.splitK; ++k) {
            const float4 v = *reinterpret_cast<const float4*>(src + (size_t)k * slice);
            s.x += v.x; s.y += v.y; s.z += v.z; s.w += v.w;
        }
        store_quad<E>(a, p, co, s.x, s.y, s.z, s.w);
    }
}

template <typename E, int TC, int TP, int WC, int WP, int PD, int KWID>
int launch_pd(const ConvArgs& a0, hipStream_t s) {
    ConvArgs a = a0;
    a.nPixTiles = cdiv(a.P, TP);
    a.nCoTiles = cdiv(a.Cout, TC);
    const int grid = a.nPixTiles * a.nCoTiles;
    const size_t lds = 2 * (TC + TP) * 64 * KWID;
    hipLaunchKernelGGL((conv_igemm_kernel<E, TC, TP, WC, WP, PD, KWID>), dim3(grid, a.splitK), dim3(256), lds, s, a);
    FLAIR_LAUNCH_CHECK();
    if (a.splitK > 1) {
        long g = (a.P * (a.Cout / 4) + 255) / 256;
        if (g > 2048) g = 2048;
        hipLaunchKernelGGL(conv_splitk_reduce_kernel<E>, dim3((int)g), dim3(256), 0, s, a);
        FLAIR_LAUNCH_CHECK();
    }
    return FLAIR_OK;
}

template <typename E, int TC, int TP, int WC, int WP>
int launch(const ConvArgs& a, hipStream_t s) {
    if constexpr (sizeof(E) == 2) {
        bool ok = true;
        for (int i = 0; i < a.nseg; ++i) ok = ok && a.segC[i] % 64 == 0;
        if (ok) return launch_pd<E, TC, TP, WC, WP, 2, 2>(a, s);
    }
    return launch_pd<E, TC, TP, WC, WP, 4, 1>(a, s);
}

int choose_split(const ConvArgs& a, int variant) {
    if (variant > 2) return 1;
    const int maxBlocks = variant == 0 ? 512 : 1024, maxSplit = 16;
    const int tc = variant == 0 ? 128 : 64, tp = variant == 2 ? 64 : 128;
    const int bke = 64 / (a.wBytes && a.CinTot ? (int)(a.wBytes / ((unsigned long long)a.Cout * a.KT * a.KH * a.KW * a.CinTot)) : 2);
    const long nk = (long)a.KT * a.KH * a.KW * (a.CinTot / bke);
    const long tiles = (long)cdiv(a.P, tp) * cdiv(a.Cout, tc);
    if (tiles >= 384 || nk < 32) return 1;
    long s = maxBlocks / tiles;
    if (s > maxSplit) s = maxSplit;
    if (s > nk / 8) s = nk / 8;
    return s < 1 ? 1 : (int)s;
}

int choose_variant(const ConvArgs& a) {
    if (!a.reflect && a.stride == 1 && a.KH == 3 && a.KW == 3 && a.W % 32 == 0 && a.H >= 2) {
        const long per = (long)a.T * (a.W / 32) * cdiv(a.Cout, 64);
        const bool ks = a.Cout % 8 == 0;
        if (a.esz == 2 && ks && a.act != FLAIR_ACT_GELU && a.H % 16 == 0 && per * cdiv(a.H, 8) > 256 && per * (a.H / 16) >= 192) return 8;
        const bool dmaOk = a.esz == 2 && ks && a.act != FLAIR_ACT_GELU;
        if (per * cdiv(a.H, 8) >= 256) return ks && per * cdiv(a.H, 8) <= 256 ? (dmaOk && a.H % 8 == 0 ? 9 : 6) : 3;
        if (per * cdiv(a.H, 4) >= 256) return ks && per * cdiv(a.H, 4) <= 256 ? 7 : 4;
        return 5;
    }
    const long tiles128 = (long)cdiv(a.P, 128) * cdiv(a.Cout, 128);
    if (a.Cout > 64 && tiles128 >= 512) return 0;
    if (a.Cout >= 128 && a.P >= 1024 && tiles128 <= 64 && (long)a.KT * a.KH * a.KW * a.CinTot >= 2304) return 0;
    const long tiles64x128 = (long)cdiv(a.P, 128) * cdiv(a.Cout, 64);
    if (tiles64x128 >= 512) return 1;
    return 2;
}

template <typename E>
int dispatch(const ConvArgs& a0, hipStream_t s) {
    ConvArgs a = a0;
    const int variant = choose_variant(a);
    a.splitK = a.part ? choose_split(a, variant) : 1;
    switch (variant) {
        case 0: return launch<E, 128, 128, 2, 2>(a, s);
        case 1: return launch<E, 64, 128, 1, 4>(a, s);
        case 2: return launch<E, 64, 64, 2, 2>(a, s);
        case 3: return launch_halo<E, 8, 1, 1>(a, s);
        case 4: return launch_halo<E, 4, 1, 1>(a, s);
        case 6: return launch_halo_ks<E, 8, 1, 2>(a, s);
        case 7: return launch_halo_ks<E, 4, 1, 2>(a, s);
        case 8: return launch_dma<8, 2, 2>(a, s);
        case 9:
            if (frame_kernel_ok(a)) return launch_frame(a, s);
            return launch_dma<8, 1, 2>(a, s);
        default: return launch_halo<E, 2, 1, 1>(a, s);
    }
}

}

extern "C" int flair_conv_variant(const flair_conv_params* p);

static void fill_geometry(ConvArgs& a, const flair_conv_params* p) {
    a.stride = p->stride > 1 ? p->stride : 1;
    a.Hin = p->H; a.Win = p->W;
    a.T = p->T; a.KT = p->KT; a.KH = p->KH; a.KW = p->KW; a.Cout = p->Cout;
    a.reflect = p->reflect_pad ? 1 : 0;
    a.act = p->act;
    a.H = (p->H + a.stride - 1) / a.stride;
    a.W = (p->W + a.stride - 1) / a.stride;
    a.P = (long)p->T * a.H * a.W;
    a.CinTot = 0;
    for (int i = 0; i < p->nseg && i < 4; ++i) a.CinTot += p->seg_c[i];
    const int esz = p->dtype == FLAIR_BF16 ? 2 : 4;
    a.esz = esz;
    a.wBytes = (unsigned)((unsigned long long)p->Cout * p->KT * p->KH * p->KW * a.CinTot * esz);
}

extern "C" size_t flair_conv_workspace_bytes(const flair_conv_params* p) {
    if (!p) return 0;
    ConvArgs a{};
    fill_geometry(a, p);
    const int split = choose_split(a, choose_variant(a));
    return split > 1 ? (size_t)split * a.P * a.Cout * sizeof(float) : 0;
}

extern "C" int flair_conv_nhwc(const flair_conv_params* p, const void* const* x, const void* w,
                               const float* bias, const float* frame_bias, const void* res0, const void* res1,
                               void* y, void* workspace, size_t workspace_bytes, hipStream_t stream) {
    FLAIR_CHECK(p && x && w && y, "flair_conv_nhwc: null argument");
    FLAIR_CHECK(p->dtype == FLAIR_F32 || p->dtype == FLAIR_BF16, "flair_conv_nhwc: bad dtype %d", p->dtype);
    FLAIR_CHECK(p->nseg >= 1 && p->nseg <= 4, "flair_conv_nhwc: nseg %d not in 1..4", p->nseg);
    FLAIR_CHECK(p->T > 0 && p->H > 0 && p->W > 0 && p->Cout > 0, "flair_conv_nhwc: empty shape");
    FLAIR_CHECK((p->KT & 1) && (p->KH & 1) && (p->KW & 1), "flair_conv_nhwc: kernel taps must be odd");
    FLAIR_CHECK(p->Cout % 4 == 0, "flair_conv_nhwc: Cout %d must be a multiple of 4", p->Cout);
    const int bke = p->dtype == FLAIR_BF16 ? 32 : 16;
    const int esz = p->dtype == FLAIR_BF16 ? 2 : 4;
    ConvArgs a{};
    a.CinTot = 0;
    for (int i = 0; i < p->nseg; ++i) {
        FLAIR_CHECK(x[i], "flair_conv_nhwc: segment %d is null", i);
        FLAIR_CHECK(p->seg_c[i] > 0 && p->seg_c[i] % bke == 0,
                    "flair_conv_nhwc: segment %d has %d channels; must be a multiple of %d", i, p->seg_c[i], bke);
        FLAIR_CHECK(p->seg_ld[i] >= p->seg_c[i] && (p->seg_ld[i] * esz) % 16 == 0 &&
                        ((uintptr_t)x[i]) % 16 == 0,
                    "flair_conv_nhwc: segment %d stride/alignment", i);
        a.x[i] = x[i];
        a.segC[i] = p->seg_c[i];
        a.segLd[i] = p->seg_ld[i];
        a.CinTot += p->seg_c[i];
        const unsigned long long bytes = (unsigned long long)p->H * p->W * p->seg_ld[i] * esz;
        FLAIR_CHECK(bytes < 0x40000000ull, "flair_conv_nhwc: one frame of segment %d spans %llu bytes (limit 1 GiB)",
                    i, bytes);
        a.segBytes[i] = (unsigned)bytes;
    }
    {
        const unsigned long long wb = (unsigned long long)p->Cout * p->KT * p->KH * p->KW * a.CinTot * esz;
        FLAIR_CHECK(wb < 0x80000000ull, "flair_conv_nhwc: weights span %llu bytes (limit 2 GiB)", wb);
        a.wBytes = (unsigned)wb;
    }
    const int gran = (p->dtype == FLAIR_BF16 && p->Cout % 8 != 0) ? 8 : 16;
    FLAIR_CHECK(p->y_ld >= p->Cout && (p->y_ld * esz) % gran == 0 && ((uintptr_t)y) % 16 == 0,
                "flair_conv_nhwc: output stride/alignment (y_ld = %d: >= Cout = %d, a multiple of %d bytes; y 16-byte aligned)",
                p->y_ld, p->Cout, gran);
    FLAIR_CHECK(!res0 || (p->res_ld[0] >= p->Cout && (p->res_ld[0] * esz) % gran == 0 && ((uintptr_t)res0) % gran == 0),
                "flair_conv_nhwc: res0 stride/alignment (res_ld = %d: >= Cout = %d; stride and pointer multiples of %d bytes)",
                p->res_ld[0], p->Cout, gran);
    FLAIR_CHECK(!res1 || (p->res_ld[1] >= p->Cout && (p->res_ld[1] * esz) % gran == 0 && ((uintptr_t)res1) % gran == 0),
                "flair_conv_nhwc: res1 stride/alignment (res_ld = %d: >= Cout = %d; stride and pointer multiples of %d bytes)",
                p->res_ld[1], p->Cout, gran);
    FLAIR_CHECK(((uintptr_t)w) % 16 == 0, "flair_conv_nhwc: weight alignment");
    FLAIR_CHECK(!bias || ((uintptr_t)bias) % 16 == 0, "flair_conv_nhwc: bias alignment");
    a.nseg = p->nseg;
    a.w = w;
    a.bias = bias;
    a.fbias = frame_bias;
    a.fbiasLd = p->frame_bias_ld;
    FLAIR_CHECK(!frame_bias || p->frame_bias_ld >= p->Cout, "flair_conv_nhwc: frame_bias_ld");
    {
        const unsigned long long hw = (unsigned long long)p->H * p->W * esz;
        FLAIR_CHECK(hw * p->y_ld < 0x40000000ull && (!res0 || hw * p->res_ld[0] < 0x40000000ull) && (!res1 || hw * p->res_ld[1] < 0x40000000ull),
                    "flair_conv_nhwc: one frame of the output / a residual spans more than 1 GiB");
    }
    a.res0 = res0;
    a.res1 = res1;
    a.res0Ld = p->res_ld[0];
    a.res1Ld = p->res_ld[1];
    a.y = y;
    a.yLd = p->y_ld;
    a.act = p->act;
    a.actParam = p->act_param;
    a.actPeriod = p->act_period;
    FLAIR_CHECK(p->act != FLAIR_ACT_DCN_OFFSETS || (p->act_period > 0 && p->act_period % 24 == 0),
                "flair_conv_nhwc: FLAIR_ACT_DCN_OFFSETS needs act_period = 3 * deform_groups (multiple of 24), got %d",
                p->act_period);
    a.outScale = p->out_scale;
    {
        ConvArgs g{};
        fill_geometry(g, p);
        a.stride = g.stride; a.Hin = g.Hin; a.Win = g.Win; a.T = g.T; a.H = g.H; a.W = g.W; a.P = g.P;
        a.KT = g.KT; a.KH = g.KH; a.KW = g.KW; a.Cout = g.Cout; a.esz = g.esz;
    }
    FLAIR_CHECK(a.stride == 1 || a.stride == 2, "flair_conv_nhwc: stride %d unsupported", p->stride);
    FLAIR_CHECK(!p->asym_pad || (a.stride == 2 && a.KH == a.KW && a.KT == 1 && p->H % 2 == 0 && p->W % 2 == 0),
                "flair_conv_nhwc: asym_pad needs a square 2-D stride-2 kernel on even frames");
    a.tapShift = p->asym_pad ? a.KH / 2 : 0;
    FLAIR_CHECK(!p->reflect_pad || (!p->asym_pad && a.KT == 1 && p->H > a.KH / 2 && p->W > a.KW / 2),
                "flair_conv_nhwc: reflect_pad needs a 2-D kernel smaller than the frame");
    a.reflect = p->reflect_pad ? 1 : 0;
    a.part = nullptr;
    a.splitK = 1;

    if (workspace && workspace_bytes >= flair_conv_workspace_bytes(p) && flair_conv_workspace_bytes(p) > 0) {
        FLAIR_CHECK(((uintptr_t)workspace) % 16 == 0, "flair_conv_nhwc: workspace alignment");
        a.part = reinterpret_cast<float*>(workspace);
    }
    if (p->dtype == FLAIR_BF16) return dispatch<bf16_t>(a, stream);
    return dispatch<float>(a, stream);
}

extern "C" int flair_conv_variant(const flair_conv_params* p) {
    if (!p) return -1;
    ConvArgs a{};
    fill_geometry(a, p);
    return choose_variant(a);
}
```

flair_amd/csrc/warp.hip:

```cpp
#include "common.h"

namespace {

__device__ __forceinline__ float gs_coord(float pix, int size) {
    const float denom = (float)(size > 1 ? size - 1 : 1);
    const float g = 2.0f * pix / denom - 1.0f;
    float r = ((g + 1.f) / 2.f) * (float)(size - 1);
    asm("" : "+v"(r));
    return r;
}

template <typename E>
__global__ void flow_warp_kernel(const E* x, int xLd, const float* flow, int fLd, int F, int H, int W, int C, int border,
                                 E* y, int yLd) {
    constexpr int VEC = ET<E>::VEC;
    const int cv = C / VEC;
    const long total = (long)F * H * W * cv;
    const __amdgpu_buffer_rsrc_t xr = make_rsrc(x, (unsigned)((size_t)F * H * W * xLd * sizeof(E)));
    for (long i = blockIdx.x * (long)blockDim.x + threadIdx.x; i < total; i += (long)gridDim.x * blockDim.x) {
        const int c0 = (int)(i % cv) * VEC;
        const long p = i / cv;
        const int w = (int)(p % W);
        const int h = (int)((p / W) % H);
        const long f = p / ((long)W * H);
        const float2 fl = *reinterpret_cast<const float2*>(flow + p * fLd);
        float ix = gs_coord((float)w + fl.x, W);
        float iy = gs_coord((float)h + fl.y, H);
        if (border) {
            ix = fminf(fmaxf(ix, 0.f), (float)(W - 1));
            iy = fminf(fmaxf(iy, 0.f), (float)(H - 1));
        }
        const float fx = floorf(ix), fy = floorf(iy);
        const int x0 = (int)fx, y0 = (int)fy;
        const float ax = ix - fx, ay = iy - fy;
        const float wgt[4] = {(1.f - ax) * (1.f - ay), ax * (1.f - ay), (1.f - ax) * ay, ax * ay};
        uint4 cq[4];
#pragma unroll
        for (int q = 0; q < 4; ++q) {
            const int xx = x0 + (q & 1), yy = y0 + (q >> 1);
            const bool in = (unsigned)xx < (unsigned)W && (unsigned)yy < (unsigned)H;
            cq[q] = buf_load16(xr, in ? (unsigned)(((f * H + yy) * W + xx) * xLd + c0) * (unsigned)sizeof(E) : FLAIR_OOB);
        }
        float acc[VEC];
#pragma unroll
        for (int k = 0; k < VEC; ++k) acc[k] = 0.f;
#pragma unroll
        for (int q = 0; q < 4; ++q) {
            float v[VEC];
            Vec16<E>::load(reinterpret_cast<const E*>(&cq[q]), v);
#pragma unroll
            for (int k = 0; k < VEC; ++k) acc[k] = fmaf(wgt[q], v[k], acc[k]);
        }
        Vec16<E>::store(y + p * yLd + c0, acc);
    }
}

__global__ void flow_compose_kernel(const float* f1, const float* f2, int F, int H, int W, float* out) {
    const long total = (long)F * H * W;
    for (long p = blockIdx.x * (long)blockDim.x + threadIdx.x; p < total; p += (long)gridDim.x * blockDim.x) {
        const int w = (int)(p % W);
        const int h = (int)((p / W) % H);
        const long f = p / ((long)W * H);
        const float2 fl = *reinterpret_cast<const float2*>(f1 + p * 2);
        const float ix = gs_coord((float)w + fl.x, W), iy = gs_coord((float)h + fl.y, H);
        const float fx = floorf(ix), fy = floorf(iy);
        const int x0 = (int)fx, y0 = (int)fy;
        const float ax = ix - fx, ay = iy - fy;
        const float wgt[4] = {(1.f - ax) * (1.f - ay), ax * (1.f - ay), (1.f - ax) * ay, ax * ay};
        float ox = 0.f, oy = 0.f;
#pragma unroll
        for (int q = 0; q < 4; ++q) {
            const int xx = x0 + (q & 1), yy = y0 + (q >> 1);
            if ((unsigned)xx < (unsigned)W && (unsigned)yy < (unsigned)H) {
                const float2 v = *reinterpret_cast<const float2*>(f2 + ((f * H + yy) * W + xx) * 2);
                ox = fmaf(wgt[q], v.x, ox);
                oy = fmaf(wgt[q], v.y, oy);
            }
        }
        *reinterpret_cast<float2*>(out + p * 2) = make_float2(fl.x + ox, fl.y + oy);
    }
}


__device__ __forceinline__ void bil_setup(float px, float py, int W, int H, int (&xy)[2], float (&wgt)[4]) {
    const float ix = gs_coord(px, W), iy = gs_coord(py, H);
    const float fx = floorf(ix), fy = floorf(iy);
    xy[0] = (int)fminf(fmaxf(fx, -2.f), (float)W);
    xy[1] = (int)fminf(fmaxf(fy, -2.f), (float)H);
    const float ax = ix - fx, ay = iy - fy;
    wgt[0] = (1.f - ax) * (1.f - ay); wgt[1] = ax * (1.f - ay); wgt[2] = (1.f - ax) * ay; wgt[3] = ax * ay;
}

template <typename E>
__global__ void vsrpp_prep_kernel(const E* prop, int propLd, const E* feat2, int feat2Ld, const float* flow1,
                                  const float* flowPrev, int H, int W, int C, E* cond1, int cond1Ld, E* cond2,
                                  int cond2Ld, float* flow2Out, E* flowpad, int padLd) {
    constexpr int VEC = ET<E>::VEC;
    const int cv = C / VEC;
    const long total = (long)H * W * cv;
    for (long i = blockIdx.x * (long)blockDim.x + threadIdx.x; i < total; i += (long)gridDim.x * blockDim.x) {
        const int c0 = (int)(i % cv) * VEC;
        const long p = i / cv;
        const int w = (int)(p % W), h = (int)(p / W);
        const float2 f1 = *reinterpret_cast<const float2*>(flow1 + p * 2);
        int xy[2];
        float wg[4];
        bil_setup((float)w + f1.x, (float)h + f1.y, W, H, xy, wg);
        float acc[VEC];
#pragma unroll
        for (int k = 0; k < VEC; ++k) acc[k] = 0.f;
        float2 f2 = make_float2(0.f, 0.f);
#pragma unroll
        for (int q = 0; q < 4; ++q) {
            const int xx = xy[0] + (q & 1), yy = xy[1] + (q >> 1);
            if ((unsigned)xx < (unsigned)W && (unsigned)yy < (unsigned)H) {
                float v[VEC];
                Vec16<E>::load(prop + ((long)yy * W + xx) * propLd + c0, v);
#pragma unroll
                for (int k = 0; k < VEC; ++k) acc[k] = fmaf(wg[q], v[k], acc[k]);
                if (flowPrev) {
                    const float2 fp = *reinterpret_cast<const float2*>(flowPrev + ((long)yy * W + xx) * 2);
                    f2.x = fmaf(wg[q], fp.x, f2.x);
                    f2.y = fmaf(wg[q], fp.y, f2.y);
                }
            }
        }
        Vec16<E>::store(cond1 + p * cond1Ld + c0, acc);
        if (flowPrev) {
            f2.x += f1.x;
            f2.y += f1.y;
            bil_setup((float)w + f2.x, (float)h + f2.y, W, H, xy, wg);
#pragma unroll
            for (int k = 0; k < VEC; ++k) acc[k] = 0.f;
#pragma unroll
            for (int q = 0; q < 4; ++q) {
                const int xx = xy[0] + (q & 1), yy = xy[1] + (q >> 1);
                if ((unsigned)xx < (unsigned)W && (unsigned)yy < (unsigned)H) {
                    float v[VEC];
                    Vec16<E>::load(feat2 + ((long)yy * W + xx) * feat2Ld + c0, v);
#pragma unroll
                    for (int k = 0; k < VEC; ++k) acc[k] = fmaf(wg[q], v[k], acc[k]);
                }
            }
            Vec16<E>::store(cond2 + p * cond2Ld + c0, acc);
        }
        if (c0 == 0) {
            if (flowPrev) *reinterpret_cast<float2*>(flow2Out + p * 2) = f2;
            ET<E>::st(flowpad + p * padLd + 0, f1.x);
            ET<E>::st(flowpad + p * padLd + 1, f1.y);
            ET<E>::st(flowpad + p * padLd + 2, f2.x);
            ET<E>::st(flowpad + p * padLd + 3, f2.y);
        }
    }
}

template <typename E>
__global__ void vsrpp_warp2_kernel(const E* prop, int propLd, const E* feat2, int feat2Ld, const float* flow1,
                                   const float* flow2, int H, int W, int C, E* cond1, int cond1Ld, E* cond2,
                                   int cond2Ld) {
    prefetch_kernargs<96>();
    constexpr int VEC = ET<E>::VEC;
    const int cv = C / VEC;
    const long total = (long)H * W * cv;
    const bool second = blockIdx.y == 1;
    const E* src = second ? feat2 : prop;
    const int srcLd = second ? feat2Ld : propLd;
    const float* flow = second ? flow2 : flow1;
    E* dst = second ? cond2 : cond1;
    const int dstLd = second ? cond2Ld : cond1Ld;
    const __amdgpu_buffer_rsrc_t sr = make_rsrc(src, (unsigned)((size_t)H * W * srcLd * sizeof(E)));
    for (unsigned i = blockIdx.x * blockDim.x + threadIdx.x; i < (unsigned)total; i += gridDim.x * blockDim.x) {
        const unsigned p = i / (unsigned)cv;
        const int c0 = (int)(i - p * (unsigned)cv) * VEC;
        const int h = (int)(p / (unsigned)W), w = (int)(p - (unsigned)h * (unsigned)W);
        const float2 f = *reinterpret_cast<const float2*>(flow + (size_t)p * 2);
        int xy[2];
        float wg[4];
        bil_setup((float)w + f.x, (float)h + f.y, W, H, xy, wg);
        uint4 cq[4];
#pragma unroll
        for (int q = 0; q < 4; ++q) {
            const int xx = xy[0] + (q & 1), yy = xy[1] + (q >> 1);
            const bool in = (unsigned)xx < (unsigned)W && (unsigned)yy < (unsigned)H;
            cq[q] = buf_load16(sr, in ? (unsigned)((yy * W + xx) * srcLd + c0) * (unsigned)sizeof(E) : FLAIR_OOB);
        }
        float acc[VEC];
#pragma unroll
        for (int k = 0; k < VEC; ++k) acc[k] = 0.f;
#pragma unroll
        for (int q = 0; q < 4; ++q) {
            float v[VEC];
            Vec16<E>::load(reinterpret_cast<const E*>(&cq[q]), v);
#pragma unroll
            for (int k = 0; k < VEC; ++k) acc[k] = fmaf(wg[q], v[k], acc[k]);
        }
        Vec16<E>::store(dst + (size_t)p * dstLd + c0, acc);
    }
}

__device__ __forceinline__ float cubic1(float x, float A) { return ((A + 2.f) * x - (A + 3.f)) * x * x + 1.f; }
__device__ __forceinline__ float cubic2(float x, float A) { return ((A * x - 5.f * A) * x + 8.f * A) * x - 4.f * A; }

template <typename E>
__global__ void nearest2x_kernel(const E* x, int xLd, long F, int Hi, int Wi, int C, E* y, int yLd) {
    constexpr int VEC = ET<E>::VEC;
    const int cv = C / VEC;
    const int Ho = 2 * Hi, Wo = 2 * Wi;
    const long total = F * Ho * Wo * cv;
    for (long i = blockIdx.x * (long)blockDim.x + threadIdx.x; i < total; i += (long)gridDim.x * blockDim.x) {
        const int c = (int)(i % cv) * VEC;
        const long p = i / cv;
        const int wo = (int)(p % Wo);
        const int ho = (int)((p / Wo) % Ho);
        const long f = p / ((long)Wo * Ho);
        *reinterpret_cast<uint4*>(y + p * yLd + c) =
            *reinterpret_cast<const uint4*>(x + ((f * Hi + (ho >> 1)) * Wi + (wo >> 1)) * xLd + c);
    }
}

template <typename E>
__global__ void bilinear_vec_kernel(const E* x, int xLd, long F, int Hi, int Wi, int C, int Ho, int Wo, E* y, int yLd) {
    constexpr int VEC = ET<E>::VEC;
    const int cv = C / VEC;
    const long total = F * Ho * Wo * cv;
    const float sx = (float)Wi / (float)Wo, sy = (float)Hi / (float)Ho;
    for (long i = blockIdx.x * (long)blockDim.x + threadIdx.x; i < total; i += (long)gridDim.x * blockDim.x) {
        const int c = (int)(i % cv) * VEC;
        const long p = i / cv;
        const int wo = (int)(p % Wo);
        const int ho = (int)((p / Wo) % Ho);
        const long f = p / ((long)Wo * Ho);
        const E* fb = x + f * Hi * Wi * xLd + c;
        const float rx = fmaxf(sx * ((float)wo + 0.5f) - 0.5f, 0.f);
        const float ry = fmaxf(sy * ((float)ho + 0.5f) - 0.5f, 0.f);
        const int x0 = (int)rx, y0 = (int)ry;
        const int x1 = x0 + (x0 < Wi - 1 ? 1 : 0), y1 = y0 + (y0 < Hi - 1 ? 1 : 0);
        const float ax = rx - (float)x0, ay = ry - (float)y0;
        float v00[VEC], v01[VEC], v10[VEC], v11[VEC], r[VEC];
        Vec16<E>::load(fb + ((long)y0 * Wi + x0) * xLd, v00);
        Vec16<E>::load(fb + ((long)y0 * Wi + x1) * xLd, v01);
        Vec16<E>::load(fb + ((long)y1 * Wi + x0) * xLd, v10);
        Vec16<E>::load(fb + ((long)y1 * Wi + x1) * xLd, v11);
#pragma unroll
        for (int e = 0; e < VEC; ++e)
// ... 222 lines not shown
```

flair_amd/guided_diffusion/unet_new.py:

```python
import math

import torch
import torch.nn as nn

from .. import ops
from .nn_new import conv_nd, linear, normalization, zero_module

A = ops


class PlaceHolder(nn.Module):

    def __init__(self, module):
        super().__init__()
        self.wrapped_module = module


LazyReshaper2D = LazyReshaper3D = PlaceHolder


class TemporalWrapper(PlaceHolder):
    """unet_new.py:50-59 (skipped when ``enable_cross_frames`` is False)."""


# ... 144 lines not shown
        self._pk = dict(
            g=_dev(self.norm.wrapped_module.weight, device), be=_dev(self.norm.wrapped_module.bias, device),
            wqkv=_pack(self.qkv.weight.unsqueeze(-1), [(c, c)], dtype, device), bqkv=_dev(self.qkv.bias, device),
            wp=_pack(self.proj_out.weight.unsqueeze(-1), [(c, c)], dtype, device),
            bp=_dev(self.proj_out.bias, device))

    def run(self, ctx, x):
        pk, c = self._pk, self.channels
        n = ops.group_norm(x, pk["g"], pk["be"], eps=self.norm.wrapped_module.eps)
        qkv = ops.conv(n, pk["wqkv"], pk["bqkv"], 3 * c, (1, 1, 1))
        a = ops.qkv_attention(qkv, self.num_heads, new_order=self.new_order)
        if self.bottleneck:
            ops.add_frame_bias(a, ctx.film_all[:, self.film_off:self.film_off + c])
        return ops.conv(a, pk["wp"], pk["bp"], c, (1, 1, 1), res0=x)


class AttentionbottleBlock(AttentionBlock):

    bottleneck = True


class FalshAttn(nn.Module):
    """nn.py:389-394 -- marker only (the window attention kernel replaces flash-attn)."""


class TemporalAttention(nn.Module):

    def __init__(self, channels, num_frames, num_heads=1, num_head_channels=-1, use_checkpoint=False):
        super().__init__()
        self.channels = channels
        if num_head_channels == -1:
            self.num_heads = num_heads
        else:
            assert channels % num_head_channels == 0
            self.num_heads = channels // num_head_channels
        assert num_frames % 2 == 1, "num_frames must be odd"
        self.head_dim = temporal_head_width(channels, self.num_heads)
        self.num_frames = num_frames
        self.q_linear = linear(channels, channels)
        self.k_linear = linear(channels, channels)
        self.v_linear = linear(channels, channels)
        self.attn = FalshAttn()
        self.proj = zero_module(PlaceHolder(conv_nd(2, channels, channels, 1)))
        self.norm = PlaceHolder(normalization(channels))
        self._pk = None

    def pack(self, dtype, device):
        c, f = self.channels, self.num_frames
        offs = torch.arange(f, dtype=torch.float32, device=device) - f // 2
        mid = f // 2
        wq, wk, wv = (_dev(m.weight, device) for m in (self.q_linear, self.k_linear, self.v_linear))
        if torch.device(device).type == "cuda":
            pe = ops.timestep_embedding(offs, c)
            bq = ops.linear(pe[mid:mid + 1].contiguous(), wq, _dev(self.q_linear.bias, device))
            kpos = ops.linear(torch.cat([pe[:mid], pe[mid + 1:]]).contiguous(), wk, None)
        else:
            freqs = torch.exp(-math.log(10000.0) * torch.arange(c // 2, dtype=torch.float32) / (c // 2))
            ang = offs[:, None] * freqs[None]
            pe = torch.cat([torch.cos(ang), torch.sin(ang)], dim=-1)
            bq = pe[mid:mid + 1] @ wq.t() + _dev(self.q_linear.bias, device)
            kpos = torch.cat([pe[:mid], pe[mid + 1:]]) @ wk.t()
        wqkv = torch.cat([wq, wk, wv]).reshape(3 * c, c, 1, 1)
        bqkv = torch.cat([bq.reshape(-1), _dev(self.k_linear.bias, device), _dev(self.v_linear.bias, device)])
        self._pk = dict(
            g=_dev(self.norm.wrapped_module.weight, device), be=_dev(self.norm.wrapped_module.bias, device),
            wqkv=_pack(wqkv, [(c, c)], dtype, device), bqkv=bqkv.contiguous(), kpos=kpos,
            wp=_pack(self.proj.wrapped_module.weight, [(c, c)], dtype, device),
            bp=_dev(self.proj.wrapped_module.bias, device))

    def run(self, ctx, h):
        pk, c = self._pk, self.channels
        n = ops.group_norm(h, pk["g"], pk["be"], eps=self.norm.wrapped_module.eps)
        qkv = ops.conv(n, pk["wqkv"], pk["bqkv"], 3 * c, (1, 1, 1))
        a = ops.temporal_attention(qkv, pk["kpos"], self.num_frames,
                                   round_fp16=(ctx.dtype == torch.float32), head_dim=self.head_dim)
        return ops.conv(a, pk["wp"], pk["bp"], c, (1, 1, 1), res0=h)


class ResidualBlockNoBN(nn.Module):
    def __init__(self, mid_channels):
        super().__init__()
        self.conv1 = nn.Conv2d(mid_channels, mid_channels, 3, 1, 1, bias=True)
        self.conv2 = nn.Conv2d(mid_channels, mid_channels, 3, 1, 1, bias=True)


class ResidualBlocksWithInputConv(nn.Module):

    def __init__(self, in_channels, out_channels=64, num_blocks=1):
        super().__init__()
        if num_blocks != 1:
            raise NotImplementedError("flair_amd: FLAIR uses one residual block per trunk")
        self.main = nn.Sequential(nn.Conv2d(in_channels, out_channels, 3, 1, 1, bias=True),
                                  nn.LeakyReLU(negative_slope=0.1),
                                  nn.Sequential(ResidualBlockNoBN(out_channels)))

    def pack(self, dtype, device, split):
        c = self.main[0].out_channels
        rb = self.main[2][0]
        return dict(w0=_pack(self.main[0].weight, [(s, s) for s in split], dtype, device),
                    b0=_dev(self.main[0].bias, device),
                    w1=_pack(rb.conv1.weight, [(c, c)], dtype, device), b1=_dev(rb.conv1.bias, device),
                    w2=_pack(rb.conv2.weight, [(c, c)], dtype, device), b2=_dev(rb.conv2.bias, device))




def run_trunk(pk, segs, c, *, extra_res=None, out=None, out_scale=1.0):
    k = (1, 3, 3)
    t1 = ops.conv(segs, pk["w0"], pk["b0"], c, k, act=A.ACT_LRELU01)
    if c == 64 and ops.chain_supported(t1, c):
        return ops.conv_chain(t1, pk["w1"], pk["b1"], A.ACT_RELU, pk["w2"], pk["b2"], A.ACT_NONE, c, c,
                              res0=t1, res1=extra_res, out=out, out_scale=out_scale)
    t2 = ops.conv(t1, pk["w1"], pk["b1"], c, k, act=A.ACT_RELU)
    return ops.conv(t2, pk["w2"], pk["b2"], c, k, res0=t1, res1=extra_res, out=out, out_scale=out_scale)


class SecondOrderDeformableAlignment(nn.Module):

    def __init__(self, in_channels, out_channels, kernel_size=3, padding=1, deform_groups=16,
                 max_residue_magnitude=10):
        super().__init__()
        assert kernel_size == 3 and padding == 1
        self.in_channels, self.out_channels = in_channels, out_channels
        self.deform_groups, self.max_residue_magnitude = deform_groups, max_residue_magnitude
        self.weight = nn.Parameter(torch.empty(out_channels, in_channels, 3, 3))
        self.bias = nn.Parameter(torch.zeros(out_channels))
        stdv = 1.0 / math.sqrt(in_channels * 9)
        with torch.no_grad():
            self.weight.uniform_(-stdv, stdv)
        c = out_channels
        self.conv_offset = nn.Sequential(
            nn.Conv2d(3 * c + 4, c, 3, 1, 1), nn.LeakyReLU(negative_slope=0.1),
            nn.Conv2d(c, c, 3, 1, 1), nn.LeakyReLU(negative_slope=0.1),
            nn.Conv2d(c, c, 3, 1, 1), nn.LeakyReLU(negative_slope=0.1),
            nn.Conv2d(c, 27 * deform_groups, 3, 1, 1))
        zero_module(self.conv_offset[-1])

    def pack(self, dtype, device):
        c = self.out_channels
        ka = ops.k_align(dtype)
        co = self.conv_offset
        perm = ops.dcn_raw_permutation(self.deform_groups)
        w6, b6 = co[6].weight.detach()[perm], co[6].bias.detach()[perm]
        return dict(
            w0=_pack(co[0].weight, [(c, c), (c, c), (c, c), (4, ka)], dtype, device), b0=_dev(co[0].bias, device),
            w2=_pack(co[2].weight, [(c, c)], dtype, device), b2=_dev(co[2].bias, device),
            w4=_pack(co[4].weight, [(c, c)], dtype, device), b4=_dev(co[4].bias, device),
            w6=_pack(w6, [(c, c)], dtype, device), b6=_dev(b6, device),
            wd=_pack(self.weight, [(2 * c, 2 * c)], dtype, device), bd=_dev(self.bias, device))


class BasicVSRPP(nn.Module):

    def __init__(self, mid_channels=64, max_residue_magnitude=10, use_checkpoint=False):
        super().__init__()
        self.mid_channels = mid_channels
        self.deform_align = nn.ModuleDict()
        self.backbone = nn.ModuleDict()
        for i, name in enumerate(["backward_1", "forward_1"]):
            self.deform_align[name] = SecondOrderDeformableAlignment(
                2 * mid_channels, mid_channels, 3, padding=1, deform_groups=16,
                max_residue_magnitude=max_residue_magnitude)
            self.backbone[name] = ResidualBlocksWithInputConv((2 + i) * mid_channels, mid_channels, 1)
        self.reconstruction = ResidualBlocksWithInputConv(3 * mid_channels, mid_channels, 1)
        self.conv_last = zero_module(nn.Conv2d(mid_channels, mid_channels, 1, 1))
        self._pk = None

    def pack(self, dtype, device):
        c = self.mid_channels
        self._pk = dict(
            align={n: m.pack(dtype, device) for n, m in self.deform_align.items()},
            trunk={"backward_1": self.backbone["backward_1"].pack(dtype, device, [c, c]),
                   "forward_1": self.backbone["forward_1"].pack(dtype, device, [c, c, c])},
            recon=self.reconstruction.pack(dtype, device, [c, c, c]),
            wl=_pack(self.conv_last.weight, [(c, c)], dtype, device), bl=_dev(self.conv_last.bias, device))

    def _propagate(self, ctx, hidden, flows, name, others, weight, wmaps, dest):
        pk_a, pk_t = self._pk["align"][name], self._pk["trunk"][name]
        T, H, W, c = hidden.shape
        order = list(range(T))
        flow_idx = list(range(-1, T - 1))
        if "backward" in name:
            order = order[::-1]
            flow_idx = order
        zero_c = torch.zeros((1, H, W, c), dtype=ctx.dtype, device=ctx.device)
        ka = ops.k_align(ctx.dtype)
        k3 = (1, 3, 3)
        G = self.deform_align[name].deform_groups
        mag = float(self.deform_align[name].max_residue_magnitude)
        store = ctx.flows.get("_prop") if isinstance(ctx.flows, dict) else None
        key = (name, H, W, ctx.dtype, ka)
        cached = store.get(key) if store is not None else None
        fill = [] if (cached is None and store is not None) else None
        prop, prev2 = zero_c, None
        for i, idx in enumerate(order):
            cur = hidden[idx:idx + 1]
            if i > 0:
                flow_n1 = flows[flow_idx[i]:flow_idx[i] + 1]
                cond_n1 = torch.empty_like(zero_c)
                second = i > 1
                feat_n2 = prev2 if second else zero_c
                cond_n2 = torch.empty_like(zero_c) if second else zero_c
                if cached is not None:
                    flow_n2, flowpad = cached[i - 1]
                    ops.vsrpp_warp2(prop, feat_n2 if second else None, flow_n1, flow_n2, cond_n1, cond_n2 if second else None)
                else:
                    flowpad = torch.zeros((1, H, W, ka), dtype=ctx.dtype, device=ctx.device)
                    flow_n2 = torch.empty_like(flow_n1) if second else None
                    ops.vsrpp_prep(prop, feat_n2 if second else None, flow_n1,
                                   flows[flow_idx[i - 1]:flow_idx[i - 1] + 1] if second else None,
                                   cond_n1, cond_n2 if second else None, flow_n2, flowpad)
                    if fill is not None:
                        fill.append((flow_n2, flowpad))
                o = ops.conv([cond_n1, cur, cond_n2, flowpad], pk_a["w0"], pk_a["b0"], c, k3, act=A.ACT_LRELU01)
                if c == 64 and ops.chain_supported(o, c):
                    o = ops.conv_chain(o, pk_a["w2"], pk_a["b2"], A.ACT_LRELU01, pk_a["w4"], pk_a["b4"],
                                       A.ACT_LRELU01, c, c)
                else:
                    o = ops.conv(o, pk_a["w2"], pk_a["b2"], c, k3, act=A.ACT_LRELU01)
                    o = ops.conv(o, pk_a["w4"], pk_a["b4"], c, k3, act=A.ACT_LRELU01)
                if c == 64 and ops.chain_supported(o, c) and W % 32 == 0:
                    raw = ops.conv_chain(o, None, None, A.ACT_NONE, pk_a["w6"], pk_a["b6"], A.ACT_DCN_OFFSETS, c, 27 * G,
                                         act_param=mag, act_period=3 * G)
                else:
                    raw = ops.conv(o, pk_a["w6"], pk_a["b6"], 27 * G, k3, act=A.ACT_DCN_OFFSETS, act_param=mag,
                                   act_period=3 * G)
                aligned = ops.dcn_align(prop, feat_n2, raw, flow_n1, flow_n2, pk_a["wd"], pk_a["bd"], c,
                                        groups=G, max_mag=mag, raw_activated=True)

            else:
                aligned = zero_c
            segs = [cur] + [o_[idx:idx + 1] for o_ in others] + [aligned]
            new = run_trunk(pk_t, segs, c, extra_res=aligned, out=dest[idx:idx + 1], out_scale=weight)
            if wmaps is not None:
                ops.scale_pixels(new, wmaps[idx])
            prev2, prop = (prop if i > 0 else None), new
        if fill is not None:
            store[key] = fill
        return dest

    def run(self, ctx, hidden):
        T, H, W, c = hidden.shape
        flows_forward, flows_backward = ctx.flows[W]
        weight, wmaps = 1.0, None
        vw = ctx.vsrpp_weights
        if isinstance(vw, (float, int)):
            weight = float(vw)
        elif vw is not None:
            wm = vw.reshape(T, vw.shape[-2], vw.shape[-1], 1).float().contiguous()
            if wm.shape[1] != H or wm.shape[2] != W:
                wm = ops.resize(wm, (H, W), ops.RESIZE_NEAREST)
            wmaps = [wm[i] for i in range(T)]
        bwd = torch.empty_like(hidden)
        fwd = torch.empty_like(hidden)
        self._propagate(ctx, hidden, flows_backward, "backward_1", [], weight, wmaps, bwd)
        ff = flows_forward if flows_forward is not None else flows_backward.flip(0)
        self._propagate(ctx, hidden, ff, "forward_1", [bwd], weight, wmaps, fwd)
        rec = run_trunk(self._pk["recon"], [hidden, bwd, fwd], c)
        return ops.conv(rec, self._pk["wl"], self._pk["bl"], c, (1, 1, 1), res0=hidden)


class _ConvModule(nn.Module):
    def __init__(self, cin, cout):
        super().__init__()
        self.conv = nn.Conv2d(cin, cout, kernel_size=7, stride=1, padding=3)


class SPyNetBasicModule(nn.Module):
    def __init__(self):
        super().__init__()
        ch = [8, 32, 64, 32, 16, 2]
        self.basic_module = nn.Sequential(*[_ConvModule(ch[i], ch[i + 1]) for i in range(5)])


class SPyNet(nn.Module):

    def __init__(self, pretrained=None):
        super().__init__()
        self.basic_module = nn.ModuleList([SPyNetBasicModule() for _ in range(6)])
        self.register_buffer("mean", torch.tensor([0.485, 0.456, 0.406]).view(1, 3, 1, 1))
        self.register_buffer("std", torch.tensor([0.229, 0.224, 0.225]).view(1, 3, 1, 1))
        self._pk = None

    def pack(self, device):
        f32 = torch.float32
        levels = []
        for bm in self.basic_module:
            convs = [m.conv for m in bm.basic_module]
            ws = [_pack(convs[0].weight, [(3, 4), (3, 4), (2, 8)], f32, device)]
            ws += [_pack(convs[j].weight, [(convs[j].in_channels,) * 2], f32, device) for j in (1, 2, 3)]
            ws.append(_pack(convs[4].weight, [(16, 16)], f32, device, cout_pad=4))
            bs = [_dev(convs[j].bias, device) for j in range(4)]
            bs.append(torch.cat([_dev(convs[4].bias, device), torch.zeros(2, device=device)]).contiguous())
            levels.append((ws, bs))
        mean = _dev(self.mean.reshape(-1), device)
        istd = (1.0 / _dev(self.std.reshape(-1), device)).contiguous()
        self._pk = dict(levels=levels, mean=mean, istd=istd)

    def run(self, ref, supp):
        F_, h0, w0, _ = ref.shape
        dev = ref.device
        if F_ == 0:
            return torch.zeros((0, h0, w0, 2), dtype=torch.float32, device=dev)
        h = h0 if h0 % 32 == 0 else 32 * (h0 // 32 + 1)
        w = w0 if w0 % 32 == 0 else 32 * (w0 // 32 + 1)
        if (h, w) != (h0, w0):
            ref = ops.resize(ref, (h, w), ops.RESIZE_BILINEAR, channels=3)
            supp = ops.resize(supp, (h, w), ops.RESIZE_BILINEAR, channels=3)
        sizes = [(h >> (5 - l), w >> (5 - l)) for l in range(6)]
        bufs = [torch.zeros((F_, *sizes[l], 16), dtype=torch.float32, device=dev) for l in range(6)]
        sp = [None] * 6
        ops.cast_channels(ref[..., :3], bufs[5], 0)
        sp[5] = supp
        for l in range(4, -1, -1):
            ops.resize(bufs[l + 1][..., 0:4], sizes[l], ops.RESIZE_AVGPOOL2, channels=3, out=bufs[l][..., 0:4])
            sp[l] = ops.resize(sp[l + 1], sizes[l], ops.RESIZE_AVGPOOL2, channels=3)
        flow = None
        k7 = (1, 7, 7)
        for l in range(6):
            b = bufs[l]
            if l > 0:
                ops.resize(flow, sizes[l], ops.RESIZE_BILINEAR_AC, channels=2, out=b[..., 8:12],
                           scale_c0=2.0, scale_c1=2.0)
            ops.flow_warp(sp[l], b[..., 8:10], border=True, out=b[..., 4:8])
            ws, bs = self._pk["levels"][l]
            y = ops.conv(b, ws[0], bs[0], 32, k7, act=A.ACT_RELU)
            y = ops.conv(y, ws[1], bs[1], 64, k7, act=A.ACT_RELU)
            y = ops.conv(y, ws[2], bs[2], 32, k7, act=A.ACT_RELU)
            y = ops.conv(y, ws[3], bs[3], 16, k7, act=A.ACT_RELU)
            flow = ops.conv(y, ws[4], bs[4], 4, k7, res0=b[..., 8:12])
        out = torch.empty((F_, h0, w0, 2), dtype=torch.float32, device=dev)
        ops.resize(flow, (h0, w0), ops.RESIZE_BILINEAR, channels=2, out=out,
                   scale_c0=float(w0) / float(w), scale_c1=float(h0) / float(h))
        return out


class TimestepEmbedSequential(nn.Sequential):

    def run(self, ctx, h, skip=None):
        for i, layer in enumerate(self):
            inner = layer.wrapped_module if isinstance(layer, PlaceHolder) else layer
            if isinstance(layer, TemporalWrapper) and not ctx.enable_cross_frames:
                continue
            if isinstance(inner, ResBlock):
                h = inner.run(ctx, h, skip if i == 0 else None)
            elif isinstance(inner, (AttentionBlock, TemporalAttention, BasicVSRPP)):
                h = inner.run(ctx, h)
            elif isinstance(inner, nn.Conv2d):
                h = ops.conv(h, inner._pk_w, inner._pk_b, inner.out_channels, (1, 3, 3))
            elif isinstance(inner, nn.Identity):
                pass
            else:
                raise TypeError(f"flair_amd: no executor for {type(inner).__name__}")
        return h


class UNetModel(nn.Module):

    def __init__(self, image_size, in_channels, model_channels, out_channels, num_res_blocks,
                 attention_resolutions, rnn_resolutions, dropout=0, channel_mult=(1, 2, 4, 8),
                 conv_resample=True, dims=2, num_classes=None, use_checkpoint=False, use_fp16=False,
                 num_heads=1, num_head_channels=-1, num_heads_upsample=-1, use_scale_shift_norm=False,
                 resblock_updown=False, use_new_attention_order=False, temporal_block=False):
        super().__init__()
        if dims != 2 or num_classes is not None or not resblock_updown:
            raise NotImplementedError("flair_amd: UNetModel covers the FLAIR video configuration "
                                      "(dims=2, resblock_updown=True, no class conditioning)")
# ... 269 lines not shown
```

flair_amd/ops.py:

```python
import ctypes

import torch

from . import _lib
from ._lib import (ACT_DCN_OFFSETS, ACT_GELU, ACT_LRELU01, ACT_LRELU02, ACT_NONE, ACT_RELU, ACT_SILU, ConvParams, check, dtype_code, lib,
                   ptr, stream)

__all__ = ["conv", "conv_chain", "group_norm", "nchw_to_clip", "clip_to_nchw", "timestep_embedding", "linear",
           "qkv_attention", "temporal_attention", "flow_warp", "flow_compose", "resize",
           "dcn_align", "dcn_raw_permutation", "scale_pixels", "predict_xstart", "sampler_update",
           "ACT_NONE", "ACT_RELU", "ACT_LRELU01", "ACT_SILU", "ACT_DCN_OFFSETS", "ACT_LRELU02", "ACT_GELU"]


class GnParams(ctypes.Structure):
    _fields_ = [("dtype", ctypes.c_int), ("C", ctypes.c_int), ("c0", ctypes.c_int),
                ("ld0", ctypes.c_int), ("ld1", ctypes.c_int), ("groups", ctypes.c_int),
                ("F", ctypes.c_int), ("H", ctypes.c_int), ("W", ctypes.c_int),
                ("frames_per_stat", ctypes.c_int), ("eps", ctypes.c_float), ("act", ctypes.c_int),
                ("resample", ctypes.c_int), ("y_ld", ctypes.c_int), ("raw_ld", ctypes.c_int),
                ("film_ld", ctypes.c_int)]


class SamplerCoefs(ctypes.Structure):
    _fields_ = [("gamma", ctypes.c_float), ("w_aux", ctypes.c_float),
                ("sqrt_recip_alphas_cumprod", ctypes.c_float),
                ("sqrt_recipm1_alphas_cumprod", ctypes.c_float),
                ("sqrt_alphas_cumprod_prev", ctypes.c_float),
                ("sqrt_one_minus_alphas_cumprod_prev", ctypes.c_float),
                ("sqrt_one_minus_rho", ctypes.c_float), ("sqrt_rho", ctypes.c_float),
                ("clip_denoised", ctypes.c_int), ("nonzero", ctypes.c_int),
                ("frame_elems", ctypes.c_long), ("frames", ctypes.c_int),
                ("prev_frames", ctypes.c_int)]


class AttnParams(ctypes.Structure):
    _fields_ = [("dtype", ctypes.c_int), ("frames", ctypes.c_int), ("L", ctypes.c_int),
                ("heads", ctypes.c_int), ("head_dim", ctypes.c_int), ("ld", ctypes.c_int),
                ("out_ld", ctypes.c_int), ("q_off", ctypes.c_int), ("k_off", ctypes.c_int),
                ("v_off", ctypes.c_int), ("head_stride", ctypes.c_int), ("scale", ctypes.c_float)]


class TAttnParams(ctypes.Structure):
    _fields_ = [("dtype", ctypes.c_int), ("T", ctypes.c_int), ("H", ctypes.c_int),
                ("W", ctypes.c_int), ("C", ctypes.c_int), ("window", ctypes.c_int),
                ("ld", ctypes.c_int), ("out_ld", ctypes.c_int), ("round_fp16", ctypes.c_int),
                ("scale", ctypes.c_float), ("head_dim", ctypes.c_int)]


class DcnParams(ctypes.Structure):
    _fields_ = [("dtype", ctypes.c_int), ("F", ctypes.c_int), ("H", ctypes.c_int),
                ("W", ctypes.c_int), ("Cin", ctypes.c_int), ("Cout", ctypes.c_int),
                ("G", ctypes.c_int), ("x_ld", ctypes.c_int * 2), ("raw_ld", ctypes.c_int),
                ("y_ld", ctypes.c_int), ("max_residue_magnitude", ctypes.c_float), ("raw_activated", ctypes.c_int)]


def _ld(t):
    assert t.dim() == 4 and t.stride(3) == 1, "clip tensors are (T,H,W,C) with C innermost"
    ld = t.stride(2)
    assert t.stride(1) == ld * t.shape[2] and (t.shape[0] == 1 or t.stride(0) == ld * t.shape[1] * t.shape[2]), \
        "clip tensor must be dense over (T,H,W)"
    return ld


def _f32(t):
    assert t is None or (t.dtype == torch.float32 and t.is_contiguous())
    return t


def k_align(dtype):
    return 32 if dtype == torch.bfloat16 else 16


def pad_channels(c, dtype):
    g = k_align(dtype)
    return (c + g - 1) // g * g


def conv(xs, weight, bias, cout, kernel, *, out=None, act=ACT_NONE, res0=None, res1=None,
         out_scale=1.0, stride=1, frame_bias=None, act_param=0.0, act_period=0, asym_pad=False, reflect_pad=False):
    if isinstance(xs, torch.Tensor):
        xs = [xs]
    x0 = xs[0]
    T, H, W, _ = x0.shape
    p = ConvParams()
    p.dtype = dtype_code(x0)
    p.T, p.H, p.W = T, H, W
    p.KT, p.KH, p.KW = kernel
    p.Cout = cout
    p.nseg = len(xs)
    arr = (ctypes.c_void_p * 4)()
    for i, x in enumerate(xs):
        assert x.dtype == x0.dtype and x.shape[:3] == x0.shape[:3]
        p.seg_c[i] = x.shape[3]
        p.seg_ld[i] = _ld(x)
        arr[i] = x.data_ptr()
    p.stride = stride
    p.asym_pad = int(asym_pad)
    p.reflect_pad = int(reflect_pad)
    p.frame_bias_ld = frame_bias.stride(0) if frame_bias is not None else 0
    if frame_bias is not None:
        assert frame_bias.dtype == torch.float32 and frame_bias.stride(1) == 1 and frame_bias.shape[0] == T
    Ho, Wo = (H + stride - 1) // stride, (W + stride - 1) // stride
    if out is None:
        out = torch.empty((T, Ho, Wo, cout), dtype=x0.dtype, device=x0.device)
    assert tuple(out.shape[:3]) == (T, Ho, Wo) and out.shape[3] >= cout and out.dtype == x0.dtype
    p.y_ld = _ld(out)
    p.res_ld[0] = _ld(res0) if res0 is not None else 0
    p.res_ld[1] = _ld(res1) if res1 is not None else 0
    p.act = act
    p.act_param, p.act_period = act_param, act_period
    p.out_scale = out_scale
    assert weight.dtype == x0.dtype and weight.is_contiguous()
    e0 = _prof_begin()
    wsb = _conv_ws_bytes(p)
    ws = _workspace(wsb, x0.device, "conv") if wsb else None

    def launch(_keep=xs):
        check(lib().flair_conv_nhwc(ctypes.byref(p), arr, ptr(weight), ptr(_f32(bias)), ptr(frame_bias), ptr(res0),
                                    ptr(res1), ptr(out), ptr(ws), ctypes.c_size_t(wsb), stream()), "flair_conv_nhwc")
    launch()
    if e0 is not None:
        cin = sum(x.shape[3] for x in xs)
        taps = kernel[0] * kernel[1] * kernel[2]
        esz = x0.element_size()
        flops = 2.0 * T * Ho * Wo * cout * cin * taps
        nbytes = esz * (cin * T * H * W + cout * T * Ho * Wo * (1 + (res0 is not None) + (res1 is not None))
                        + cout * taps * cin)
        _prof_end(e0, ("conv", lib().flair_conv_variant(ctypes.byref(p))), x0.dtype, flops, nbytes, launch,
                  ("conv", T, H, W, tuple(x.shape[3] for x in xs), cout, tuple(kernel), stride, act,
                   res0 is not None, res1 is not None, frame_bias is not None))
    return out


PROFILE = None


def _prof_begin():
    if PROFILE is None:
        return None
    e0 = torch.cuda.Event(enable_timing=True)
    e0.record()
    return e0


def _prof_end(e0, family, dtype, flops, nbytes, replay=None, sig=None):
    e1 = torch.cuda.Event(enable_timing=True)
    e1.record()
    PROFILE.append((family, str(dtype), float(flops), float(nbytes), e0, e1, replay, sig))


def conv_variant(T, H, W, cins, cout, kernel, dtype=torch.bfloat16, stride=1):
    p = ConvParams()
    p.dtype = 1 if dtype == torch.bfloat16 else 0
    p.T, p.H, p.W = T, H, W
    p.KT, p.KH, p.KW = kernel
    p.Cout = cout
    p.nseg = len(cins)
    for i, c in enumerate(cins):
        p.seg_c[i] = c
        p.seg_ld[i] = c
    p.stride = stride
    p.y_ld = cout
    return lib().flair_conv_variant(ctypes.byref(p))


def _conv_ws_bytes(p):
    f = lib().flair_conv_workspace_bytes
    f.restype = ctypes.c_size_t
    return f(ctypes.byref(p))


def pack_conv_weight(w, seg_channels, dtype, cout_pad=None):
    cout, cin = w.shape[:2]
    taps = 1
    for k in w.shape[2:]:
        taps *= k
    w = w.reshape(cout, cin, taps).permute(0, 2, 1).float()
    parts, o = [], 0
    for real, padded in seg_channels:
        seg = w[:, :, o:o + real]
        if padded > real:
            seg = torch.cat([seg, seg.new_zeros(cout, taps, padded - real)], dim=2)
        parts.append(seg)
        o += real
    assert o == cin, (o, cin)
    w = torch.cat(parts, dim=2)
    if cout_pad is not None and cout_pad > cout:
        w = torch.cat([w, w.new_zeros(cout_pad - cout, taps, w.shape[2])], dim=0)
    return w.to(dtype).contiguous()


class ChainParams(ctypes.Structure):
    _fields_ = [("dtype", ctypes.c_int), ("T", ctypes.c_int), ("H", ctypes.c_int), ("W", ctypes.c_int),
                ("C", ctypes.c_int), ("CoutB", ctypes.c_int), ("nseg", ctypes.c_int),
                ("seg_c", ctypes.c_int * 4), ("seg_ld", ctypes.c_int * 4), ("y_ld", ctypes.c_int),
                ("res_ld", ctypes.c_int * 2), ("actA", ctypes.c_int), ("actB", ctypes.c_int),
                ("out_scale", ctypes.c_float), ("act_param", ctypes.c_float), ("act_period", ctypes.c_int)]


def chain_supported(xs, c_mid):
    x0 = xs[0] if isinstance(xs, (list, tuple)) else xs
    T, H, W, _ = x0.shape
    tiles = T * ((H + 7) // 8) * (W // 32 if W % 32 == 0 and T * ((H + 7) // 8) * (W // 32) >= 192 else W // 8)
    return c_mid in (64, 128) and W % 8 == 0 and tiles <= 512


def conv_chain(xs, wA, bA, actA, wB, bB, actB, c_mid, coutB, *, res0=None, res1=None, out_scale=1.0, out=None,
               act_param=0.0, act_period=0):
    if isinstance(xs, torch.Tensor):
        xs = [xs]
    x0 = xs[0]
    T, H, W, _ = x0.shape
    p = ChainParams()
    p.dtype = dtype_code(x0)
    p.T, p.H, p.W = T, H, W
    p.C, p.CoutB = c_mid, coutB
    p.nseg = len(xs)
    arr = (ctypes.c_void_p * 4)()
    for i, x in enumerate(xs):
        assert x.dtype == x0.dtype and x.shape[:3] == x0.shape[:3]
        p.seg_c[i] = x.shape[3]
        p.seg_ld[i] = _ld(x)
        arr[i] = x.data_ptr()
    if out is None:
        out = torch.empty((T, H, W, coutB), dtype=x0.dtype, device=x0.device)
    assert tuple(out.shape[:3]) == (T, H, W) and out.shape[3] >= coutB and out.dtype == x0.dtype
    p.y_ld = _ld(out)
    p.res_ld[0] = _ld(res0) if res0 is not None else 0
    p.res_ld[1] = _ld(res1) if res1 is not None else 0
    p.actA, p.actB = actA, actB
    p.act_param, p.act_period = act_param, act_period
    p.out_scale = out_scale
    assert wB.dtype == x0.dtype and wB.is_contiguous() and (wA is None or (wA.dtype == x0.dtype and wA.is_contiguous()))
    e0 = _prof_begin()

    def launch(_keep=xs):
        check(lib().flair_conv_chain(ctypes.byref(p), arr, ptr(wA), ptr(_f32(bA)), ptr(wB), ptr(_f32(bB)), ptr(res0),
                                     ptr(res1), ptr(out), stream()), "flair_conv_chain")
    launch()
    if e0 is not None:
        cin = sum(x.shape[3] for x in xs)
        esz = x0.element_size()
        px = T * H * W
        flops = 2.0 * 9 * px * (c_mid * coutB + (cin * c_mid if wA is not None else 0))
        nbytes = esz * (px * (cin + coutB * (1 + (res0 is not None) + (res1 is not None)))
                        + 9 * c_mid * coutB + (9 * cin * c_mid if wA is not None else 0))
        _prof_end(e0, ("chain", 2 if wA is not None else 1, c_mid), x0.dtype, flops, nbytes, launch,
                  ("chain", T, H, W, tuple(x.shape[3] for x in xs), c_mid, coutB, wA is not None, res0 is not None,
                   res1 is not None))
    return out


_gn_ws = {}


def _workspace(nbytes, device, tag="gn"):
    key = (tag, device, torch.cuda.current_stream().cuda_stream)
    buf = _gn_ws.get(key)
    if buf is None or buf.numel() < nbytes:
        buf = torch.empty(max(nbytes, 1 << 20), dtype=torch.uint8, device=device)
        _gn_ws[key] = buf
    return buf


def group_norm(x, gamma, beta, *, x1=None, groups=32, eps=1e-5, act=ACT_NONE, film=None,
               frames_per_stat=None, resample=0, out=None, want_raw=False):
    T, H, W, c0 = x.shape
    C = c0 + (x1.shape[3] if x1 is not None else 0)
    p = GnParams()
    p.dtype = dtype_code(x)
    p.C, p.c0 = C, c0
    p.ld0 = _ld(x)
    p.ld1 = _ld(x1) if x1 is not None else 0
    p.groups = groups
    p.F, p.H, p.W = T, H, W
    p.frames_per_stat = frames_per_stat or T
    p.eps = eps
    p.act = act
    p.resample = resample
    Ho, Wo = (H // 2, W // 2) if resample == 1 else ((H * 2, W * 2) if resample == 2 else (H, W))
    if out is None:
        out = torch.empty((T, Ho, Wo, C), dtype=x.dtype, device=x.device)
    raw = torch.empty((T, Ho, Wo, C), dtype=x.dtype, device=x.device) if want_raw else None
    p.y_ld = _ld(out)
    p.raw_ld = _ld(raw) if raw is not None else 0
    p.film_ld = film.stride(0) if film is not None else 0
# ... 577 lines not shown
```

include/flair_hip.h:

```cpp
#ifndef FLAIR_HIP_H
#define FLAIR_HIP_H

#include <stddef.h>
#include <stdint.h>

#ifdef __cplusplus
extern "C" {
#endif

#ifndef __HIP_PLATFORM_AMD__
typedef struct ihipStream_t* hipStream_t;
#endif

typedef enum {
    FLAIR_OK = 0,
    FLAIR_ERR_ARG = -1,
    FLAIR_ERR_HIP = -2
} flair_status;

typedef enum { FLAIR_F32 = 0, FLAIR_BF16 = 1 } flair_dtype;

typedef enum {
    FLAIR_ACT_NONE = 0,
    FLAIR_ACT_RELU = 1,
    FLAIR_ACT_LRELU01 = 2,
    FLAIR_ACT_SILU = 3,
    FLAIR_ACT_DCN_OFFSETS = 4,
    FLAIR_ACT_LRELU02 = 5,
    FLAIR_ACT_GELU = 6
} flair_act;

const char* flair_last_error(void);
int flair_abi_version(void);

typedef struct {
    int dtype;
    int T, H, W;
    int KT, KH, KW;
    int Cout;
    int nseg;
    int seg_c[4];
    int seg_ld[4];
    int y_ld;
    int res_ld[2];
    int act;
    float out_scale;
    int frame_bias_ld;
    int stride;
    float act_param;
    int act_period;
    int asym_pad;
    int reflect_pad;
} flair_conv_params;

size_t flair_conv_workspace_bytes(const flair_conv_params* p);
int flair_conv_nhwc(const flair_conv_params* p, const void* const* x, const void* w,
                    const float* bias, const float* frame_bias, const void* res0, const void* res1,
                    void* y, void* workspace, size_t workspace_bytes, hipStream_t stream);
int flair_conv_variant(const flair_conv_params* p);


typedef struct {
    int dtype;
    int T, H, W;
    int C;
    int CoutB;
    int nseg;
    int seg_c[4];
    int seg_ld[4];
    int y_ld;
    int res_ld[2];
    int actA, actB;
    float out_scale;
    float act_param;
    int act_period;
} flair_chain_params;

int flair_conv_chain(const flair_chain_params* p, const void* const* x, const void* wA, const float* biasA,
                     const void* wB, const float* biasB, const void* res0, const void* res1, void* y,
                     hipStream_t stream);


typedef struct {
    int dtype;
    int C, c0;
    int ld0, ld1;
    int groups;
    int F, H, W;
    int frames_per_stat;
    float eps;
    int act;
    int resample;
    int y_ld, raw_ld;
    int film_ld;
} flair_gn_params;

size_t flair_groupnorm_workspace_bytes(const flair_gn_params* p);
int flair_groupnorm_nhwc(const flair_gn_params* p, const void* x0, const void* x1,
                         const float* gamma, const float* beta, const float* film, void* y,
                         void* raw, void* workspace, hipStream_t stream);

int flair_nchw_f32_to_nhwc(const float* src, int N, int C, int H, int W, void* dst, int dtype,
                           int dst_ld, int dst_coff, hipStream_t stream);
int flair_nhwc_to_nchw_f32(const void* src, int dtype, int src_ld, int src_coff, int N, int C,
                           int H, int W, float* dst, hipStream_t stream);

int flair_timestep_embedding(const float* t, int N, int dim, float max_period, int sin_first,
                             float* out, hipStream_t stream);

int flair_linear_f32(const float* x, int M, int K, const float* w, const float* bias, int N,
                     int act_in, int act_out, float* y, int y_ld, hipStream_t stream);

typedef struct {
    float gamma, w_aux;
    float sqrt_recip_alphas_cumprod, sqrt_recipm1_alphas_cumprod;
    float sqrt_alphas_cumprod_prev, sqrt_one_minus_alphas_cumprod_prev;
    float sqrt_one_minus_rho, sqrt_rho;
    int clip_denoised, nonzero;
    long frame_elems;
    int frames, prev_frames;
} flair_sampler_coefs;

int flair_predict_xstart(const float* x, const float* model_out, int N, int C, int Cm, int H, int W,
                         float c_recip, float c_recipm1, int clip, float* x0, hipStream_t stream);
int flair_sampler_update(const flair_sampler_coefs* c, const float* x, float* x0,
                         const float* restored, const float* aux, const float* z,
                         const float* prev_recon, long n, float* x_prev, hipStream_t stream);
int flair_axpby_f32(const float* x, const float* y, float a, float b, float lo, float hi, long n,
                    float* out, hipStream_t stream);
int flair_learned_range_variance(const float* model_out, int N, int C, int H, int W, float min_log,
                                 float max_log, float* variance, float* log_variance,
                                 hipStream_t stream);
int flair_affine_channels_f32(const float* x, int x_ld, int C, long P, float a, float b, float lo,
                              float hi, const float* sub, const float* mul, float* y, int y_ld,
                              hipStream_t stream);
int flair_gated_blend(const void* x, int x_ld, const void* m, int m_ld, const float* gate, int gate_ld,
                      int dtype, int C, int F, long HW, void* y, int y_ld, hipStream_t stream);
int flair_add_act_nhwc(const void* x0, int x0_ld, const void* x1, int x1_ld, int dtype, int C, long P,
                       int act, void* y, int y_ld, hipStream_t stream);
int flair_maxpool3x3s2_nhwc(const void* x, int x_ld, int dtype, int F, int H, int W, int C, void* y,
                            int y_ld, hipStream_t stream);
int flair_dwconv_nhwc(const float* x, int x_ld, int T, int H, int W, int C, int stride, const float* w_dw,
                      const float* b_dw, const float* w_pw, const float* b_pw, int Cout, int act, float* y,
                      int y_ld, hipStream_t stream);
int flair_dwconv7_nhwc(const void* x, int x_ld, int dtype, int T, int H, int W, int C, const float* w,
                       const float* bias, void* y, int y_ld, hipStream_t stream);
int flair_add_frame_bias(void* x, int dtype, int ld, int C, int F, long HW, const float* bias,
                         int bias_ld, hipStream_t stream);
int flair_cast_channels(const float* src, int src_ld, int C, long P, void* dst, int dtype,
                        int dst_ld, int dst_coff, hipStream_t stream);
int flair_scale_pixels(void* x, int dtype, int ld, int C, long P, const float* wmap,
                       hipStream_t stream);

typedef struct {
    int dtype;
    int frames, L, heads, head_dim;
    int ld, out_ld;
    int q_off, k_off, v_off, head_stride;
    float scale;
} flair_attn_params;
int flair_qkv_attention(const flair_attn_params* p, const void* qkv, void* out, hipStream_t stream);

typedef struct {
    int dtype;
    int T, H, W, C, window;
    int ld, out_ld;
    int round_fp16;
    float scale;
    int head_dim;
} flair_tattn_params;
int flair_temporal_attention(const flair_tattn_params* p, const void* qkv, const float* kpos,
                             void* out, hipStream_t stream);

int flair_flow_warp(const void* x, int dtype, int x_ld, const float* flow, int flow_ld, int F,
                    int H, int W, int C, int border, void* y, int y_ld, hipStream_t stream);
int flair_flow_compose(const float* f1, const float* f2, int F, int H, int W, float* out,
                       hipStream_t stream);
int flair_vsrpp_warp2(const void* prop, int prop_ld, const void* feat2, int feat2_ld, const float* flow1,
                      const float* flow2, int dtype, int H, int W, int C, void* cond1, int cond1_ld,
                      void* cond2, int cond2_ld, hipStream_t stream);
int flair_vsrpp_prep(const void* prop, int prop_ld, const void* feat2, int feat2_ld,
                     const float* flow1, const float* flow_prev, int dtype, int H, int W, int C,
                     void* cond1, int cond1_ld, void* cond2, int cond2_ld, float* flow2_out,
                     void* flowpad, int pad_ld, hipStream_t stream);
int flair_resize_nhwc(const void* x, int dtype, int x_ld, int F, int Hi, int Wi, int C, int mode,
                      int Ho, int Wo, void* y, int y_ld, float scale_c0, float scale_c1,
                      hipStream_t stream);

typedef struct {
    int dtype;
    int F, H, W;
    int Cin, Cout, G;
    int x_ld[2];
    int raw_ld, y_ld;
    float max_residue_magnitude;
    int raw_activated;
} flair_dcn_params;
int flair_dcn_align(const flair_dcn_params* p, const void* x0, const void* x1, const void* raw,
                    const float* flow1, const float* flow2, const void* w, const float* bias,
                    void* y, hipStream_t stream);

int flair_depthwise_filter(const float* x, int planes, int Hin, int Win, const float* filt, int kh,
                           int kw, int pad, int out_stride, int out_offset, int stuff,
                           int stuff_offset, int Hout, int Wout, int reflect, float* y,
                           hipStream_t stream);
int flair_jpeg_roundtrip(const float* x, int N, int S, const float* q_luma, const float* q_chroma,
                         const float* dct8, float* workspace, float* y, float* luma_q, float* chroma_q,
                         hipStream_t stream);
int flair_matmul_f32(const float* A, long a_batch_stride, const float* B, long b_batch_stride,
                     float* C, int batch, int M, int N, int K, hipStream_t stream);
int flair_gather_mac_f32(const float* x, long outer, int Lin, long inner, const int* fov,
                         const float* w, int taps, int Lout, float* y, hipStream_t stream);
// ... 39 lines not shown
```

Before: 0.9046.

## Fuse flow-warp bilinear gather into the 3x3 conv halo load for BasicVSR++ propagation

Adds gather variants of the halo-tiled and frame-wide 3x3 conv kernels. For flow-warped input segments, these sample the four bilinear corners per halo pixel and blend them in registers before writing to LDS. In the BasicVSR++ propagation step, this replaces the separate warp kernel and its intermediate warped-feature tensors when the warp cache exists and the width is 64 or 128. The cost is extra register pressure, four scattered loads per halo element instead of DMA, and serialized blend writes that change the wait/pipeline schedule.

```diff
diff --git a/flair_amd/csrc/api.hip b/flair_amd/csrc/api.hip
--- a/flair_amd/csrc/api.hip
+++ b/flair_amd/csrc/api.hip
@@ -13,7 +13,7 @@
 }
 
 extern "C" const char* flair_last_error(void) { return g_err; }
-extern "C" int flair_abi_version(void) { return 11; }
+extern "C" int flair_abi_version(void) { return 12; }
 
 #include <dlfcn.h>
 
diff --git a/flair_amd/csrc/common.h b/flair_amd/csrc/common.h
--- a/flair_amd/csrc/common.h
+++ b/flair_amd/csrc/common.h
@@ -124,6 +124,32 @@
 __device__ __forceinline__ uint4 buf_load16(__amdgpu_buffer_rsrc_t r, unsigned byteOff) {
     const u32x4_t v = __builtin_amdgcn_raw_buffer_load_b128(r, (int)byteOff, 0, 0);
     return make_uint4(v.x, v.y, v.z, v.w);
+}
+
+__device__ __forceinline__ float gs_coord(float pix, int size) {
+    const float denom = (float)(size > 1 ? size - 1 : 1);
+    const float g = 2.0f * pix / denom - 1.0f;
+    float r = ((g + 1.f) / 2.f) * (float)(size - 1);
+    asm("" : "+v"(r));
+    return r;
+}
+
+__device__ __forceinline__ void bil_coords(float px, float py, int W, int H, int (&xy)[2], float (&frac)[2]) {
+    const float ix = gs_coord(px, W), iy = gs_coord(py, H);
+    const float fx = floorf(ix), fy = floorf(iy);
+    xy[0] = (int)fminf(fmaxf(fx, -2.f), (float)W);
+    xy[1] = (int)fminf(fmaxf(fy, -2.f), (float)H);
+    frac[0] = ix - fx;
+    frac[1] = iy - fy;
+}
+__device__ __forceinline__ void bil_weights(const float (&frac)[2], float (&wgt)[4]) {
+    const float ax = frac[0], ay = frac[1];
+    wgt[0] = (1.f - ax) * (1.f - ay); wgt[1] = ax * (1.f - ay); wgt[2] = (1.f - ax) * ay; wgt[3] = ax * ay;
+}
+__device__ __forceinline__ void bil_setup(float px, float py, int W, int H, int (&xy)[2], float (&wgt)[4]) {
+    float frac[2];
+    bil_coords(px, py, W, H, xy, frac);
+    bil_weights(frac, wgt);
 }
 
 __device__ __forceinline__ int xcd_remap(int bid, int nwg) {
diff --git a/flair_amd/csrc/conv.hip b/flair_amd/csrc/conv.hip
--- a/flair_amd/csrc/conv.hip
+++ b/flair_amd/csrc/conv.hip
@@ -39,6 +39,33 @@
     int esz;
 };
 
+struct WarpArgs {
+    const float* flow[4];
+};
+
+__device__ __forceinline__ uint4 blend_corners(const uint4 (&cq)[4], const float (&wg)[4]) {
+    float acc[8];
+#pragma unroll
+    for (int k = 0; k < 8; ++k) acc[k] = 0.f;
+#pragma unroll
+    for (int q = 0; q < 4; ++q) {
+        float v[8];
+        Vec16<bf16_t>::load(reinterpret_cast<const bf16_t*>(&cq[q]), v);
+#pragma unroll
+        for (int k = 0; k < 8; ++k) acc[k] = fmaf(wg[q], v[k], acc[k]);
+    }
+    uint4 o;
+    o.x = pack2bf(acc[0], acc[1]); o.y = pack2bf(acc[2], acc[3]);
+    o.z = pack2bf(acc[4], acc[5]); o.w = pack2bf(acc[6], acc[7]);
+    return o;
+}
+
+__device__ __forceinline__ unsigned corner_off(const int (&xy)[2], int q, int W, int H, unsigned ldB, unsigned cofs, bool ok) {
+    const int xx = xy[0] + (q & 1), yy = xy[1] + (q >> 1);
+    const bool in = ok && (unsigned)xx < (unsigned)W && (unsigned)yy < (unsigned)H;
+    return in ? (unsigned)(yy * W + xx) * ldB + cofs : FLAIR_OOB;
+}
+
 template <typename E> struct Mma;
 
 template <> struct Mma<bf16_t> {
@@ -502,10 +529,11 @@
     return FLAIR_OK;
 }
 
-template <typename E, int TH, int RPW, int CF>
-__global__ __launch_bounds__(256 * TH / RPW / CF, (256 * TH / RPW / CF) / 256) void conv3x3_halo_ks_kernel(ConvArgs a) {
+template <typename E, int TH, int RPW, int CF, bool GATHER>
+__device__ __forceinline__ void conv3x3_halo_ks_body(const ConvArgs& a, const WarpArgs& g) {
     static_assert(RPW == 1 && CF == 2, "one image row and both 32-cout fragments per wave");
-    prefetch_kernargs<sizeof(ConvArgs)>();
+    static_assert(!GATHER || sizeof(E) == 2, "the gathering form is bf16");
+    prefetch_kernargs<sizeof(ConvArgs) + (GATHER ? sizeof(WarpArgs) : 0)>();
     constexpr int NRG = TH / RPW;
     constexpr int NCG = 2 / CF;
     constexpr int NW = 2 * NRG * NCG, NT = 64 * NW;
@@ -560,6 +588,32 @@
         hpix[i] = ok ? hh * a.W + ww : -1;
         hq[i] = (id & 3) * VEC * ESZ;
     }
+    constexpr int GI = GATHER ? HI : 1;
+    float2 gfl[2][GI];
+    uint4 cq[GI][4];
+    float gwg[GI][4];
+    int gxy[GI][2];
+    int gseg1 = -1;
+    bool pendGather = false;
+    if constexpr (GATHER) {
+        int gseg0 = -1;
+        for (int sg = 0; sg < a.nseg; ++sg)
+            if (g.flow[sg]) {
+                if (gseg0 < 0) gseg0 = sg;
+                else gseg1 = sg;
+            }
+#pragma unroll
+        for (int j = 0; j < 2; ++j) {
+            const int sg = j ? gseg1 : gseg0;
+            const float* fp = sg >= 0 ? g.flow[sg] : nullptr;
+            const __amdgpu_buffer_rsrc_t fr = make_rsrc(fp, fp ? (unsigned)(a.H * a.W) * 8u : 0u);
+#pragma unroll
+            for (int i = 0; i < HI; ++i) {
+                const auto v = __builtin_amdgcn_raw_buffer_load_b64(fr, (int)(hpix[i] >= 0 ? (unsigned)hpix[i] * 8u : FLAIR_OOB), 0, 0);
+                gfl[j][i] = make_float2(__uint_as_float(v[0]), __uint_as_float(v[1]));
+            }
+        }
+    }
     const __amdgpu_buffer_rsrc_t wrs = make_rsrc(a.w, a.wBytes);
 #pragma unroll
     for (int i = 0; i < WI; ++i) {
@@ -574,9 +628,30 @@
         const char* frame = reinterpret_cast<const char*>(a.x[seg]) + (size_t)(t + dt) * a.H * a.W * ld;
         const __amdgpu_buffer_rsrc_t xr = make_rsrc(frame, a.segBytes[seg]);
         const unsigned cofs = (unsigned)(cb * BKE) * ESZ;
-#pragma unroll
-        for (int i = 0; i < HI; ++i)
-            hreg[i] = buf_load16(xr, hpix[i] >= 0 ? (unsigned)hpix[i] * ld + cofs + hq[i] : FLAIR_OOB);
+        bool gather = false;
+        if constexpr (GATHER) gather = g.flow[seg] != nullptr;
+        if (gather) {
+            if constexpr (GATHER) {
+                if (cb == 0) {
+#pragma unroll
+                    for (int i = 0; i < HI; ++i) {
+                        const float2 f = seg == gseg1 ? gfl[1][i] : gfl[0][i];
+                        const int pix = hpix[i] >= 0 ? hpix[i] : 0;
+                        const int hh = pix / a.W, ww = pix - hh * a.W;
+                        bil_setup((float)ww + f.x, (float)hh + f.y, a.W, a.H, gxy[i], gwg[i]);
+                    }
+                }
+#pragma unroll
+                for (int i = 0; i < HI; ++i)
+#pragma unroll
+                    for (int q = 0; q < 4; ++q) cq[i][q] = buf_load16(xr, corner_off(gxy[i], q, a.W, a.H, ld, cofs + hq[i], hpix[i] >= 0));
+            }
+        } else {
+#pragma unroll
+            for (int i = 0; i < HI; ++i)
+                hreg[i] = buf_load16(xr, hpix[i] >= 0 ? (unsigned)hpix[i] * ld + cofs + hq[i] : FLAIR_OOB);
+        }
+        pendGather = gather;
         const unsigned kofs = (unsigned)((dt + pt) * 9 * a.CinTot + segOff + cb * BKE) * ESZ;
 #pragma unroll
         for (int i = 0; i < WI; ++i) wreg[i] = buf_load16(wrs, woff[i] == FLAIR_OOB ? FLAIR_OOB : woff[i] + kofs);
@@ -595,6 +670,12 @@
     auto write_lds = [&](int stage) {
         char* sh = smem + stage * STAGE_BYTES;
         char* sw = sh + HALO_BYTES;
+        if constexpr (GATHER) {
+            if (pendGather) {
+#pragma unroll
+                for (int i = 0; i < HI; ++i) hreg[i] = blend_corners(cq[i], gwg[i]);
+            }
+        }
 #pragma unroll
         for (int i = 0; i < HI; ++i) {
             const int id = i * NT + tid;
@@ -755,6 +836,32 @@
         for (int e = 0; e < VEC; ++e) v[e] *= a.outScale;
         Vec16<E>::store(reinterpret_cast<E*>(a.y) + p * a.yLd + eco, v);
     }
+}
+
+template <typename E, int TH, int RPW, int CF>
+__global__ __launch_bounds__(256 * TH / RPW / CF, (256 * TH / RPW / CF) / 256) void conv3x3_halo_ks_kernel(ConvArgs a) {
+    conv3x3_halo_ks_body<E, TH, RPW, CF, false>(a, WarpArgs{});
+}
+
+template <typename E, int TH, int RPW, int CF>
+__global__ __launch_bounds__(256 * TH / RPW / CF, (256 * TH / RPW / CF) / 256) void conv3x3_halo_ks_gather_kernel(ConvArgs a, WarpArgs g) {
+    conv3x3_halo_ks_body<E, TH, RPW, CF, true>(a, g);
+}
+
+template <typename E, int TH, int RPW, int CF>
+int launch_halo_ks_gather(const ConvArgs& a0, const WarpArgs& g, hipStream_t s) {
+    ConvArgs a = a0;
+    a.nCoTiles = cdiv(a.Cout, 64);
+    const int grid = a.T * cdiv(a.H, TH) * (a.W / 32) * a.nCoTiles;
+    const size_t lds = 2 * ((size_t)(TH + 2) * 34 * 80 + 64 * 9 * 80);
+    static LdsAttrOnce attr;
+    {
+        const hipError_t e = flair_max_lds_once(attr, reinterpret_cast<const void*>(&conv3x3_halo_ks_gather_kernel<E, TH, RPW, CF>));
+        FLAIR_CHECK(e == hipSuccess, "flair_conv_warped_nhwc: hipFuncSetAttribute: %s", hipGetErrorString(e));
+    }
+    hipLaunchKernelGGL((conv3x3_halo_ks_gather_kernel<E, TH, RPW, CF>), dim3(grid), dim3(256 * TH / RPW / CF), lds, s, a, g);
+    FLAIR_LAUNCH_CHECK();
+    return FLAIR_OK;
 }
 
 template <typename E, int TH, int RPW, int CF>
@@ -1225,10 +1332,10 @@
 }
 
 
-template <bool HALO3>
-__global__ __launch_bounds__(512, 2) void conv_frame_kernel(ConvArgs a) {
+template <bool HALO3, bool GATHER>
+__device__ __forceinline__ void conv_frame_body(const ConvArgs& a, const WarpArgs& g) {
     static_assert(HALO3, "halo ring of three, weight ring of two");
-    prefetch_kernargs<sizeof(ConvArgs)>();
+    prefetch_kernargs<sizeof(ConvArgs) + (GATHER ? sizeof(WarpArgs) : 0)>();
     using E = bf16_t;
     constexpr int NW = 8, HWP = 34;
     constexpr int HINSTR = 22, HIMG = HINSTR * 1024, WINSTR = 36, SLOT = WINSTR * 1024;
@@ -1260,6 +1367,36 @@
         hpix[i] = ok ? (unsigned)(hh * a.W + ww) : 0xffffffffu;
         hpiece[i] = (unsigned)((lchunk ^ ((c >> 2) & 3)) << 4);
     }
+    constexpr int GI = GATHER ? NH : 1;
+    float2 gfl[2][GI];
+    int gseg1 = -1;
+    uint4 cq[GI][4];
+    float gfr[GI][2];
+    int gxy[GI][2];
+    unsigned gmask = 0;
+    if constexpr (GATHER) {
+        int c0 = 0, gseg0 = -1;
+        for (int sg = 0; sg < a.nseg; ++sg) {
+            const int n = a.segC[sg] / 32;
+            if (g.flow[sg]) {
+                gmask |= ((1u << n) - 1u) << c0;
+                if (gseg0 < 0) gseg0 = sg;
+                else gseg1 = sg;
+            }
+            c0 += n;
+        }
+#pragma unroll
+        for (int j = 0; j < 2; ++j) {
+            const int sg = j ? gseg1 : gseg0;
+            const float* fp = sg >= 0 ? g.flow[sg] : nullptr;
+            const __amdgpu_buffer_rsrc_t fr = make_rsrc(fp, fp ? (unsigned)(a.H * a.W) * 8u : 0u);
+#pragma unroll
+            for (int i = 0; i < NH; ++i) {
+                const auto v = __builtin_amdgcn_raw_buffer_load_b64(fr, (int)(hpix[i] != 0xffffffffu ? hpix[i] * 8u : FLAIR_OOB), 0, 0);
+                gfl[j][i] = make_float2(__uint_as_float(v[0]), __uint_as_float(v[1]));
+            }
+        }
+    }
     unsigned wlane[NWS];
 #pragma unroll
     for (int i = 0; i < NWS; ++i) {
@@ -1270,18 +1407,53 @@
     int hseg = 0, hcb = 0;
     auto issue_halo = [&](int slot) {
         const unsigned ld = (unsigned)a.segLd[hseg] * 2u;
-        const u32x4_t xdesc = make_desc(reinterpret_cast<const char*>(a.x[hseg]) + (size_t)t * a.H * a.W * ld, a.segBytes[hseg]);
         const unsigned cofs = (unsigned)(hcb * 64);
-#pragma unroll
-        for (int i = 0; i < NH; ++i) {
-            const int k = (wave * NH + i) % HINSTR;
-            dma16(xdesc, hpix[i] == 0xffffffffu ? FLAIR_OOB : hpix[i] * ld + cofs + hpiece[i], (unsigned)(slot * HIMG + k * 1024));
+        bool gather = false;
+        if constexpr (GATHER) gather = g.flow[hseg] != nullptr;
+        if (gather) {
+            if constexpr (GATHER) {
+                if (hcb == 0) {
+#pragma unroll
+                    for (int i = 0; i < NH; ++i) {
+                        const float2 f = hseg == gseg1 ? gfl[1][i] : gfl[0][i];
+                        const int pix = hpix[i] != 0xffffffffu ? (int)hpix[i] : 0;
+                        const int hh = pix / a.W, ww = pix - hh * a.W;
+                        bil_coords((float)ww + f.x, (float)hh + f.y, a.W, a.H, gxy[i], gfr[i]);
+                    }
+                }
+                const __amdgpu_buffer_rsrc_t xr = make_rsrc(reinterpret_cast<const char*>(a.x[hseg]) + (size_t)t * a.H * a.W * ld, a.segBytes[hseg]);
+#pragma unroll
+                for (int i = 0; i < NH; ++i)
+#pragma unroll
+                    for (int q = 0; q < 4; ++q)
+                        cq[i][q] = buf_load16(xr, corner_off(gxy[i], q, a.W, a.H, ld, cofs + hpiece[i], hpix[i] != 0xffffffffu));
+            }
+        } else {
+            const u32x4_t xdesc = make_desc(reinterpret_cast<const char*>(a.x[hseg]) + (size_t)t * a.H * a.W * ld, a.segBytes[hseg]);
+#pragma unroll
+            for (int i = 0; i < NH; ++i) {
+                const int k = (wave * NH + i) % HINSTR;
+                dma16(xdesc, hpix[i] == 0xffffffffu ? FLAIR_OOB : hpix[i] * ld + cofs + hpiece[i], (unsigned)(slot * HIMG + k * 1024));
+            }
         }
         if (++hcb * 32 >= a.segC[hseg]) {
             hcb = 0;
             ++hseg;
         }
     };
+    auto blend_write = [&](int slot) {
+        if constexpr (GATHER) {
+#pragma unroll
+            for (int i = 0; i < NH; ++i) {
+                const int k = (wave * NH + i) % HINSTR;
+                float wg[4];
+                bil_weights(gfr[i], wg);
+                *reinterpret_cast<uint4*>(smem + slot * HIMG + k * 1024 + lane * 16) = blend_corners(cq[i], wg);
+            }
+            asm volatile("s_waitcnt lgkmcnt(0)" ::: "memory");
+        }
+    };
+    auto gathered = [&](int n) { return GATHER && ((gmask >> n) & 1u) != 0; };
     auto issue_w = [&](int s_) {
 #pragma unroll
         for (int i = 0; i < NWS; ++i) {
@@ -1289,13 +1461,23 @@
             dma16(wdesc, wlane[i] == FLAIR_OOB ? FLAIR_OOB : wlane[i] + (unsigned)(s_ * 64), (unsigned)(RING + (s_ % WR) * SLOT + id * 1024));
         }
     };
-    issue_halo(0);
-    issue_w(0);
-    if (nS > 1) {
-        issue_halo(1);
-        issue_w(1);
-    }
-    if (nS > 2) issue_halo(2);
+    if constexpr (GATHER) {
+        issue_w(0);
+        if (nS > 1) issue_w(1);
+#pragma clang loop unroll(disable)
+        for (int n = 0; n < 3 && n < nS; ++n) {
+            issue_halo(n);
+            if (gathered(n)) blend_write(n);
+        }
+    } else {
+        issue_halo(0);
+        issue_w(0);
+        if (nS > 1) {
+            issue_halo(1);
+            issue_w(1);
+        }
+        if (nS > 2) issue_halo(2);
+    }
 
     unsigned aoff[2], boff[3][2];
 #pragma unroll
@@ -1350,10 +1532,18 @@
     for (int g = 0; g < 4; ++g) r0v[g] = r1v[g] = make_uint4(0u, 0u, 0u, 0u);
 
     for (int s_ = 0; s_ < nS; ++s_) {
-        if (s_ + 1 >= nS) asm volatile("s_waitcnt vmcnt(0)" ::: "memory");
-        else if (s_ == 0 && nS > 2) asm volatile("s_waitcnt vmcnt(%0)" ::"n"(2 * NH + NWS) : "memory");
-        else if (s_ == 0) asm volatile("s_waitcnt vmcnt(%0)" ::"n"(NH + NWS) : "memory");
-        else asm volatile("s_waitcnt vmcnt(%0)" ::"n"(NH) : "memory");
+        if constexpr (GATHER) {
+            int young = s_ + 1 < nS && !gathered(s_ + 1) ? NH : 0;
+            if (s_ == 0 && nS > 2 && !gathered(2)) young += NH;
+            if (young == 0) asm volatile("s_waitcnt vmcnt(0)" ::: "memory");
+            else if (young == NH) asm volatile("s_waitcnt vmcnt(%0)" ::"n"(NH) : "memory");
+            else asm volatile("s_waitcnt vmcnt(%0)" ::"n"(2 * NH) : "memory");
+        } else {
+            if (s_ + 1 >= nS) asm volatile("s_waitcnt vmcnt(0)" ::: "memory");
+            else if (s_ == 0 && nS > 2) asm volatile("s_waitcnt vmcnt(%0)" ::"n"(2 * NH + NWS) : "memory");
+            else if (s_ == 0) asm volatile("s_waitcnt vmcnt(%0)" ::"n"(NH + NWS) : "memory");
+            else asm volatile("s_waitcnt vmcnt(%0)" ::"n"(NH) : "memory");
+        }
         __builtin_amdgcn_s_barrier();
         if (s_ == 0) {
             const float* sb = reinterpret_cast<const float*>(smem + BIAS);
@@ -1367,7 +1557,7 @@
         }
         if (s_ >= 1 && s_ + 1 < nS) issue_w(s_ + 1);
         if (s_ >= 1 && s_ + 2 < nS) issue_halo((s_ + 2) % 3);
-        if (s_ + 1 == nS) {
+        if (!GATHER && s_ + 1 == nS) {
             if (a.res0) {
 #pragma unroll
                 for (int g = 0; g < 4; ++g) r0v[g] = buf_load16(r0d, 16 * g + 8 * lh < a.Cout ? (unsigned)lr * r0LdB + (unsigned)(32 * g + 16 * lh) : FLAIR_OOB);
@@ -1378,8 +1568,19 @@
             }
         }
         compute(s_ % WR, s_ % HR);
-    }
-
+        if (s_ >= 1 && s_ + 2 < nS && gathered(s_ + 2)) blend_write((s_ + 2) % 3);
+    }
+
+    if constexpr (GATHER) {
+        if (a.res0) {
+#pragma unroll
+            for (int g_ = 0; g_ < 4; ++g_) r0v[g_] = buf_load16(r0d, 16 * g_ + 8 * lh < a.Cout ? (unsigned)lr * r0LdB + (unsigned)(32 * g_ + 16 * lh) : FLAIR_OOB);
+        }
+        if (a.res1) {
+#pragma unroll
+            for (int g_ = 0; g_ < 4; ++g_) r1v[g_] = buf_load16(r1d, 16 * g_ + 8 * lh < a.Cout ? (unsigned)lr * r1LdB + (unsigned)(32 * g_ + 16 * lh) : FLAIR_OOB);
+        }
+    }
     const float slope = a.act == FLAIR_ACT_NONE ? 1.f : a.act == FLAIR_ACT_RELU ? 0.f : a.act == FLAIR_ACT_LRELU01 ? 0.1f : 0.2f;
     const float scale = a.outScale;
 #pragma unroll
@@ -1409,6 +1610,16 @@
             const unsigned yo = 16 * g + 8 * lh < a.Cout ? (unsigned)lr * yLdB + (unsigned)(32 * g + 16 * lh) : FLAIR_OOB;
             __builtin_amdgcn_raw_buffer_store_b128(u32x4_t{ov.x, ov.y, ov.z, ov.w}, yd, (int)yo, 0, 0);
         }
+}
+
+template <bool HALO3>
+__global__ __launch_bounds__(512, 2) void conv_frame_kernel(ConvArgs a) {
+    conv_frame_body<HALO3, false>(a, WarpArgs{});
+}
+
+template <bool HALO3>
+__global__ __launch_bounds__(512, 1) void conv_frame_gather_kernel(ConvArgs a, WarpArgs g) {
+    conv_frame_body<HALO3, true>(a, g);
 }
 
 static bool frame_kernel_ok(const ConvArgs& a) {
@@ -1426,6 +1637,16 @@
     const hipError_t e = flair_max_lds_once(attr, reinterpret_cast<const void*>(&conv_frame_kernel<true>));
     FLAIR_CHECK(e == hipSuccess, "flair_conv_nhwc: hipFuncSetAttribute: %s", hipGetErrorString(e));
     hipLaunchKernelGGL(conv_frame_kernel<true>, dim3(a.T * (a.H / 8) * (a.W / 32)), dim3(512), lds, s, a);
+    FLAIR_LAUNCH_CHECK();
+    return FLAIR_OK;
+}
+
+static int launch_frame_gather(const ConvArgs& a, const WarpArgs& g, hipStream_t s) {
+    constexpr size_t lds = (3 * 22 + 2 * 36) * 1024 + 1024;
+    static LdsAttrOnce attr;
+    const hipError_t e = flair_max_lds_once(attr, reinterpret_cast<const void*>(&conv_frame_gather_kernel<true>));
+    FLAIR_CHECK(e == hipSuccess, "flair_conv_warped_nhwc: hipFuncSetAttribute: %s", hipGetErrorString(e));
+    hipLaunchKernelGGL(conv_frame_gather_kernel<true>, dim3(a.T * (a.H / 8) * (a.W / 32)), dim3(512), lds, s, a, g);
     FLAIR_LAUNCH_CHECK();
     return FLAIR_OK;
 }
@@ -1792,9 +2013,8 @@
     return split > 1 ? (size_t)split * a.P * a.Cout * sizeof(float) : 0;
 }
 
-extern "C" int flair_conv_nhwc(const flair_conv_params* p, const void* const* x, const void* w,
-                               const float* bias, const float* frame_bias, const void* res0, const void* res1,
-                               void* y, void* workspace, size_t workspace_bytes, hipStream_t stream) {
+static int conv_fill_args(ConvArgs& a, const flair_conv_params* p, const void* const* x, const void* w, const float* bias,
+                          const float* frame_bias, const void* res0, const void* res1, void* y) {
     FLAIR_CHECK(p && x && w && y, "flair_conv_nhwc: null argument");
     FLAIR_CHECK(p->dtype == FLAIR_F32 || p->dtype == FLAIR_BF16, "flair_conv_nhwc: bad dtype %d", p->dtype);
     FLAIR_CHECK(p->nseg >= 1 && p->nseg <= 4, "flair_conv_nhwc: nseg %d not in 1..4", p->nseg);
@@ -1803,7 +2023,7 @@
     FLAIR_CHECK(p->Cout % 4 == 0, "flair_conv_nhwc: Cout %d must be a multiple of 4", p->Cout);
     const int bke = p->dtype == FLAIR_BF16 ? 32 : 16;
     const int esz = p->dtype == FLAIR_BF16 ? 2 : 4;
-    ConvArgs a{};
+    a = ConvArgs{};
     a.CinTot = 0;
     for (int i = 0; i < p->nseg; ++i) {
         FLAIR_CHECK(x[i], "flair_conv_nhwc: segment %d is null", i);
@@ -1877,7 +2097,14 @@
     a.reflect = p->reflect_pad ? 1 : 0;
     a.part = nullptr;
     a.splitK = 1;
-
+    return FLAIR_OK;
+}
+
+extern "C" int flair_conv_nhwc(const flair_conv_params* p, const void* const* x, const void* w,
+                               const float* bias, const float* frame_bias, const void* res0, const void* res1,
+                               void* y, void* workspace, size_t workspace_bytes, hipStream_t stream) {
+    ConvArgs a;
+    if (const int rc = conv_fill_args(a, p, x, w, bias, frame_bias, res0, res1, y)) return rc;
     if (workspace && workspace_bytes >= flair_conv_workspace_bytes(p) && flair_conv_workspace_bytes(p) > 0) {
         FLAIR_CHECK(((uintptr_t)workspace) % 16 == 0, "flair_conv_nhwc: workspace alignment");
         a.part = reinterpret_cast<float*>(workspace);
@@ -1892,3 +2119,57 @@
     fill_geometry(a, p);
     return choose_variant(a);
 }
+
+static int warped_form(const flair_conv_params* p, const int* warped, int* form) {
+    FLAIR_CHECK(p && warped, "flair_conv_warped_nhwc: null argument");
+    FLAIR_CHECK(p->dtype == FLAIR_BF16, "flair_conv_warped_nhwc: bf16 only (dtype %d)", p->dtype);
+    FLAIR_CHECK(p->T == 1, "flair_conv_warped_nhwc: one frame per call (T = %d)", p->T);
+    FLAIR_CHECK(p->KT == 1 && p->KH == 3 && p->KW == 3 && p->stride <= 1 && !p->asym_pad && !p->reflect_pad,
+                "flair_conv_warped_nhwc: 3x3, stride 1, zero padding only");
+    FLAIR_CHECK(p->nseg >= 1 && p->nseg <= 4, "flair_conv_warped_nhwc: nseg %d not in 1..4", p->nseg);
+    FLAIR_CHECK(p->H >= 2 && p->H < 32768 && p->W > 0 && p->W < 32768 && p->W % 32 == 0,
+                "flair_conv_warped_nhwc: H = %d, W = %d: W must be a multiple of 32 (and both below 32768)", p->H, p->W);
+    FLAIR_CHECK(p->Cout > 0 && p->Cout % 8 == 0, "flair_conv_warped_nhwc: Cout %d must be a multiple of 8", p->Cout);
+    FLAIR_CHECK(p->act == FLAIR_ACT_NONE || p->act == FLAIR_ACT_RELU || p->act == FLAIR_ACT_LRELU01 || p->act == FLAIR_ACT_LRELU02,
+                "flair_conv_warped_nhwc: activation %d (none, ReLU and LeakyReLU only)", p->act);
+    int c = 0, cin = 0, nwarped = 0;
+    for (int i = 0; i < p->nseg; ++i) {
+        cin += p->seg_c[i];
+        if (!warped[i]) continue;
+        FLAIR_CHECK(++nwarped <= 2, "flair_conv_warped_nhwc: at most two sampled segments");
+        FLAIR_CHECK(c == 0 || p->seg_c[i] == c, "flair_conv_warped_nhwc: sampled segments of %d and %d channels in one call", c, p->seg_c[i]);
+        c = p->seg_c[i];
+    }
+    if (c == 0) c = p->seg_c[0];
+    FLAIR_CHECK(c == 64 || c == 128, "flair_conv_warped_nhwc: sampled segments have 64 or 128 channels, not %d", c);
+    FLAIR_CHECK(cin / 32 <= 32, "flair_conv_warped_nhwc: %d input channels (at most 1024)", cin);
+    if (c == 64)
+        FLAIR_CHECK(p->Cout <= 64 && p->H % 8 == 0, "flair_conv_warped_nhwc: the 64-channel form needs Cout <= 64 and H %% 8 == 0 (Cout = %d, H = %d)",
+                    p->Cout, p->H);
+    if (form) *form = c;
+    return FLAIR_OK;
+}
+
+extern "C" int flair_conv_warped_supported(const flair_conv_params* p, const int* warped) {
+    return warped_form(p, warped, nullptr) == FLAIR_OK ? 1 : 0;
+}
+
+extern "C" int flair_conv_warped_nhwc(const flair_conv_params* p, const void* const* x, const float* const* flow, const void* w,
+                                      const float* bias, const void* res0, const void* res1, void* y, hipStream_t stream) {
+    FLAIR_CHECK(p && x && flow && w && y, "flair_conv_warped_nhwc: null argument");
+    int warped[4] = {0, 0, 0, 0}, form = 0;
+    for (int i = 0; i < 4 && i < p->nseg; ++i) warped[i] = flow[i] != nullptr;
+    if (const int rc = warped_form(p, warped, &form)) return rc;
+    ConvArgs a;
+    if (const int rc = conv_fill_args(a, p, x, w, bias, nullptr, res0, res1, y)) return rc;
+    WarpArgs g{};
+    for (int i = 0; i < p->nseg; ++i) {
+        FLAIR_CHECK(((uintptr_t)flow[i]) % 8 == 0, "flair_conv_warped_nhwc: flow %d alignment", i);
+        g.flow[i] = flow[i];
+    }
+    if (form == 64) {
+        FLAIR_CHECK(frame_kernel_ok(a), "flair_conv_warped_nhwc: the 64-channel form does not take these parameters");
+        return launch_frame_gather(a, g, stream);
+    }
+    return launch_halo_ks_gather<bf16_t, 4, 1, 2>(a, g, stream);
+}
diff --git a/flair_amd/csrc/warp.hip b/flair_amd/csrc/warp.hip
--- a/flair_amd/csrc/warp.hip
+++ b/flair_amd/csrc/warp.hip
@@ -1,14 +1,6 @@
 #include "common.h"
 
 namespace {
-
-__device__ __forceinline__ float gs_coord(float pix, int size) {
-    const float denom = (float)(size > 1 ? size - 1 : 1);
-    const float g = 2.0f * pix / denom - 1.0f;
-    float r = ((g + 1.f) / 2.f) * (float)(size - 1);
-    asm("" : "+v"(r));
-    return r;
-}
 
 template <typename E>
 __global__ void flow_warp_kernel(const E* x, int xLd, const float* flow, int fLd, int F, int H, int W, int C, int border,
@@ -81,15 +73,6 @@
     }
 }
 
-
-__device__ __forceinline__ void bil_setup(float px, float py, int W, int H, int (&xy)[2], float (&wgt)[4]) {
-    const float ix = gs_coord(px, W), iy = gs_coord(py, H);
-    const float fx = floorf(ix), fy = floorf(iy);
-    xy[0] = (int)fminf(fmaxf(fx, -2.f), (float)W);
-    xy[1] = (int)fminf(fmaxf(fy, -2.f), (float)H);
-    const float ax = ix - fx, ay = iy - fy;
-    wgt[0] = (1.f - ax) * (1.f - ay); wgt[1] = ax * (1.f - ay); wgt[2] = (1.f - ax) * ay; wgt[3] = ax * ay;
-}
 
 template <typename E>
 __global__ void vsrpp_prep_kernel(const E* prop, int propLd, const E* feat2, int feat2Ld, const float* flow1,
diff --git a/flair_amd/guided_diffusion/unet_new.py b/flair_amd/guided_diffusion/unet_new.py
--- a/flair_amd/guided_diffusion/unet_new.py
+++ b/flair_amd/guided_diffusion/unet_new.py
@@ -320,6 +320,8 @@
 
 class BasicVSRPP(nn.Module):
 
+    FOLD_WIDTHS = (64, 128)
+
     def __init__(self, mid_channels=64, max_residue_magnitude=10, use_checkpoint=False):
         super().__init__()
         self.mid_channels = mid_channels
@@ -365,22 +367,30 @@
             cur = hidden[idx:idx + 1]
             if i > 0:
                 flow_n1 = flows[flow_idx[i]:flow_idx[i] + 1]
-                cond_n1 = torch.empty_like(zero_c)
                 second = i > 1
                 feat_n2 = prev2 if second else zero_c
-                cond_n2 = torch.empty_like(zero_c) if second else zero_c
+                fold = None
                 if cached is not None:
                     flow_n2, flowpad = cached[i - 1]
-                    ops.vsrpp_warp2(prop, feat_n2 if second else None, flow_n1, flow_n2, cond_n1, cond_n2 if second else None)
+                    fold = [flow_n1, None, flow_n2 if second else None, None]
+                    if c not in self.FOLD_WIDTHS or not ops.conv_warped_supported([prop, cur, feat_n2, flowpad], fold, c, A.ACT_LRELU01):
+                        fold = None
+                if fold is not None:
+                    o = ops.conv_warped([prop, cur, feat_n2, flowpad], fold, pk_a["w0"], pk_a["b0"], c, act=A.ACT_LRELU01)
                 else:
-                    flowpad = torch.zeros((1, H, W, ka), dtype=ctx.dtype, device=ctx.device)
-                    flow_n2 = torch.empty_like(flow_n1) if second else None
-                    ops.vsrpp_prep(prop, feat_n2 if second else None, flow_n1,
-                                   flows[flow_idx[i - 1]:flow_idx[i - 1] + 1] if second else None,
-                                   cond_n1, cond_n2 if second else None, flow_n2, flowpad)
-                    if fill is not None:
-                        fill.append((flow_n2, flowpad))
-                o = ops.conv([cond_n1, cur, cond_n2, flowpad], pk_a["w0"], pk_a["b0"], c, k3, act=A.ACT_LRELU01)
+                    cond_n1 = torch.empty_like(zero_c)
+                    cond_n2 = torch.empty_like(zero_c) if second else zero_c
+                    if cached is not None:
+                        ops.vsrpp_warp2(prop, feat_n2 if second else None, flow_n1, flow_n2, cond_n1, cond_n2 if second else None)
+                    else:
+                        flowpad = torch.zeros((1, H, W, ka), dtype=ctx.dtype, device=ctx.device)
+                        flow_n2 = torch.empty_like(flow_n1) if second else None
+                        ops.vsrpp_prep(prop, feat_n2 if second else None, flow_n1,
+                                       flows[flow_idx[i - 1]:flow_idx[i - 1] + 1] if second else None,
+                                       cond_n1, cond_n2 if second else None, flow_n2, flowpad)
+                        if fill is not None:
+                            fill.append((flow_n2, flowpad))
+                    o = ops.conv([cond_n1, cur, cond_n2, flowpad], pk_a["w0"], pk_a["b0"], c, k3, act=A.ACT_LRELU01)
                 if c == 64 and ops.chain_supported(o, c):
                     o = ops.conv_chain(o, pk_a["w2"], pk_a["b2"], A.ACT_LRELU01, pk_a["w4"], pk_a["b4"],
                                        A.ACT_LRELU01, c, c)
diff --git a/flair_amd/ops.py b/flair_amd/ops.py
--- a/flair_amd/ops.py
+++ b/flair_amd/ops.py
@@ -6,7 +6,7 @@
 from ._lib import (ACT_DCN_OFFSETS, ACT_GELU, ACT_LRELU01, ACT_LRELU02, ACT_NONE, ACT_RELU, ACT_SILU, ConvParams, check, dtype_code, lib,
                    ptr, stream)
 
-__all__ = ["conv", "conv_chain", "group_norm", "nchw_to_clip", "clip_to_nchw", "timestep_embedding", "linear",
+__all__ = ["conv", "conv_warped", "conv_warped_supported", "conv_chain", "group_norm", "nchw_to_clip", "clip_to_nchw", "timestep_embedding", "linear",
            "qkv_attention", "temporal_attention", "flow_warp", "flow_compose", "resize",
            "dcn_align", "dcn_raw_permutation", "scale_pixels", "predict_xstart", "sampler_update",
            "ACT_NONE", "ACT_RELU", "ACT_LRELU01", "ACT_SILU", "ACT_DCN_OFFSETS", "ACT_LRELU02", "ACT_GELU"]
@@ -132,6 +132,69 @@
     return out
 
 
+def _warped_params(xs, cout, out, act, res0, res1, out_scale):
+    x0 = xs[0]
+    T, H, W, _ = x0.shape
+    p = ConvParams()
+    p.dtype = dtype_code(x0)
+    p.T, p.H, p.W = T, H, W
+    p.KT, p.KH, p.KW = 1, 3, 3
+    p.Cout = cout
+    p.nseg = len(xs)
+    arr = (ctypes.c_void_p * 4)()
+    for i, x in enumerate(xs):
+        assert x.dtype == x0.dtype and x.shape[:3] == x0.shape[:3]
+        p.seg_c[i] = x.shape[3]
+        p.seg_ld[i] = _ld(x)
+        arr[i] = x.data_ptr()
+    p.stride = 1
+    p.y_ld = _ld(out) if out is not None else cout
+    p.res_ld[0] = _ld(res0) if res0 is not None else 0
+    p.res_ld[1] = _ld(res1) if res1 is not None else 0
+    p.act = act
+    p.out_scale = out_scale
+    return p, arr
+
+
+def conv_warped_supported(xs, flows, cout, act=ACT_NONE):
+    f = getattr(lib(), "flair_conv_warped_supported", None)
+    if f is None or len(xs) > 4 or len(flows) != len(xs):
+        return False
+    p, _ = _warped_params(xs, cout, None, act, None, None, 1.0)
+    return bool(f(ctypes.byref(p), (ctypes.c_int * 4)(*[int(fl is not None) for fl in flows])))
+
+
+def conv_warped(xs, flows, weight, bias, cout, *, out=None, act=ACT_NONE, res0=None, res1=None, out_scale=1.0):
+    x0 = xs[0]
+    T, H, W, _ = x0.shape
+    assert len(flows) == len(xs)
+    if out is None:
+        out = torch.empty((T, H, W, cout), dtype=x0.dtype, device=x0.device)
+    assert tuple(out.shape[:3]) == (T, H, W) and out.shape[3] >= cout and out.dtype == x0.dtype
+    p, arr = _warped_params(xs, cout, out, act, res0, res1, out_scale)
+    farr = (ctypes.c_void_p * 4)()
+    for i, fl in enumerate(flows):
+        if fl is not None:
+            assert fl.dtype == torch.float32 and fl.is_contiguous() and tuple(fl.shape) == (1, H, W, 2)
+            farr[i] = fl.data_ptr()
+    assert weight.dtype == x0.dtype and weight.is_contiguous()
+    e0 = _prof_begin()
+
+    def launch(_keep=(xs, flows)):
+        check(lib().flair_conv_warped_nhwc(ctypes.byref(p), arr, farr, ptr(weight), ptr(_f32(bias)), ptr(res0), ptr(res1),
+                                           ptr(out), stream()), "flair_conv_warped_nhwc")
+    launch()
+    if e0 is not None:
+        cin = sum(x.shape[3] for x in xs)
+        esz = x0.element_size()
+        flops = 2.0 * T * H * W * cout * cin * 9
+        nbytes = esz * (cin * T * H * W + cout * T * H * W * (1 + (res0 is not None) + (res1 is not None)) + cout * 9 * cin)
+        _prof_end(e0, ("conv", lib().flair_conv_variant(ctypes.byref(p))), x0.dtype, flops, nbytes, launch,
+                  ("conv", T, H, W, tuple(x.shape[3] for x in xs), cout, (1, 3, 3), 1, act,
+                   res0 is not None, res1 is not None, False))
+    return out
+
+
 PROFILE = None
 
 
diff --git a/include/flair_hip.h b/include/flair_hip.h
--- a/include/flair_hip.h
+++ b/include/flair_hip.h
@@ -58,6 +58,10 @@
                     const float* bias, const float* frame_bias, const void* res0, const void* res1,
                     void* y, void* workspace, size_t workspace_bytes, hipStream_t stream);
 int flair_conv_variant(const flair_conv_params* p);
+
+int flair_conv_warped_supported(const flair_conv_params* p, const int* warped);
+int flair_conv_warped_nhwc(const flair_conv_params* p, const void* const* x, const float* const* flow, const void* w,
+                           const float* bias, const void* res0, const void* res1, void* y, hipStream_t stream);
 
 
 typedef struct {
```

Result: no change. 0.9057 (median of 6 runs) (+0.1%).
